# ElesionKyrie/Extreme-Video-Compression-With-Prediction-Using-Pre-trainded-Diffusion-Models-

Hardware: AMD Instinct MI355X
Metric: decoded frames/sec (128x128x30) at q3 (higher is better)
Workload: dtype f32

## Files before the change

### extreme-video-compression-with-prediction-using-pre-trainded-diffusion-models-_amd/build.py

```python
import os
import shutil
import subprocess
import sys
from concurrent.futures import ThreadPoolExecutor

HERE = os.path.dirname(os.path.abspath(__file__))
CSRC = os.path.join(HERE, "csrc")
LIBDIR = os.path.join(HERE, "lib")
OBJDIR = os.path.join(HERE, "build")
INCLUDE = os.path.join(os.path.dirname(HERE), "include")
HIP_SOURCES = ["conv_igemm.hip", "attention.hip", "norm.hip", "fir.hip", "elementwise.hip", "gdn.hip", "stride2.hip", "lpips.hip", "i3d.hip", "frames.hip", "noise.hip", "yuv.hip", "rate.hip", "ssim.hip", "inception.hip", "resample.hip", "tile.hip", "api.hip"]
ARCH = "gfx950"


def _newer(target, deps):
    if not os.path.exists(target):
        return True
    t = os.path.getmtime(target)
    return any(os.path.getmtime(d) > t for d in deps)


def _run(cmd):
    r = subprocess.run(cmd, capture_output=True, text=True)
    if r.returncode != 0:
        raise RuntimeError("build failed: %s\n%s\n%s" % (" ".join(cmd), r.stdout, r.stderr))


def hipcc_path():
    for c in (os.environ.get("HIPCC"), shutil.which("hipcc"), "/opt/rocm/bin/hipcc"):
        if c and os.path.exists(c):
            return c
    raise RuntimeError("hipcc not found (ROCm toolchain required to build libevc_hip.so)")


def build(force=False, verbose=False):
    os.makedirs(LIBDIR, exist_ok=True)
    os.makedirs(OBJDIR, exist_ok=True)
    headers = [os.path.join(INCLUDE, h) for h in ("evc_hip.h", "evc_rans.h")]
    hipcc = hipcc_path()
    flags = ["--offload-arch=" + ARCH, "-O3", "-std=c++17", "-fPIC", "-I", INCLUDE]
    flags += os.environ.get("EVC_HIPCC_FLAGS", "").split()

    def compile_one(src):
        s = os.path.join(CSRC, src)
        o = os.path.join(OBJDIR, src.replace(".hip", ".o"))
        if force or _newer(o, [s] + headers):
            if verbose:
                print("hipcc", src, flush=True)
            _run([hipcc] + flags + ["-c", s, "-o", o])
        return o

    with ThreadPoolExecutor(max_workers=min(6, len(HIP_SOURCES))) as ex:
        objs = list(ex.map(compile_one, HIP_SOURCES))
    hip_so = os.path.join(LIBDIR, "libevc_hip.so")
    if force or _newer(hip_so, objs):
        _run([hipcc, "--offload-arch=" + ARCH, "-shared", "-fPIC", "-o", hip_so] + objs)
    rans_src = os.path.join(CSRC, "rans.cpp")
    rans_so = os.path.join(LIBDIR, "libevc_rans.so")
    if force or _newer(rans_so, [rans_src] + headers):
        _run([shutil.which("g++") or "g++", "-O2", "-std=c++17", "-fPIC", "-shared", "-Wall", "-I", INCLUDE,
              rans_src, "-o", rans_so])
    return hip_so, rans_so


if __name__ == "__main__":
    print(build(force="--force" in sys.argv, verbose=True))
```

### extreme-video-compression-with-prediction-using-pre-trainded-diffusion-models-_amd/csrc/conv_igemm.hip

```cpp
#include <hip/hip_runtime.h>
#include <stdint.h>
#include <stdio.h>
#include "../../include/evc_hip.h"

typedef float f32x16 __attribute__((ext_vector_type(16)));
typedef __attribute__((address_space(3))) void lds_void;
typedef const __attribute__((address_space(1))) void glb_void;

#ifndef EVC_CONV_TAIL
#define EVC_CONV_TAIL 1
#endif
#ifndef EVC_CONV_TM1
#define EVC_CONV_TM1 1
#endif
#ifndef EVC_SPLIT_WIDE_TILES
#define EVC_SPLIT_WIDE_TILES 1
#endif

#ifndef EVC_SPLIT_INTERLEAVE
#define EVC_SPLIT_INTERLEAVE 5
#endif

namespace {

constexpr int BM_MAX = 128;
constexpr int KC = 16;

constexpr int MODE_PLAIN = 0, MODE_AFFINE = 1, MODE_AFFINE_SILU = 2, MODE_SILU = 3, MODE_RELU = 4;

struct ConvK {
    const float* src0; const float* src1; int C0; int C1; int ld0; int ld1;
    const float* coef_a; const float* coef_s;
    const float* w; const float* bias; const float* res; int ld_res;
    float out_scale; int act_out;
    float* out; int ld_out;
    int B, H, W, Co, CoPad, KH, KW;
    int M, HW, nchunk, nsteps, steps_per_split, splits;
    float* ws;
    float* stats;
    const float* w_hdr;
    const unsigned* in_bound;
    int tail_first, tail_splits, tail_sps, tail_rows;
    int cut_chunk;
    const float* x2_src0; const float* x2_src1; int x2_C0, x2_C1, x2_ld0, x2_ld1;
    const char* x2_w;
    const float* x2_hdr;
    const unsigned* x2_bound;
    int bound_stride, generic_epi;
};

__device__ __forceinline__ float bound_scale(unsigned bits) {
    const float b = sqrtf(__uint_as_float(bits));
    if (!(b < 3.0e38f)) return __builtin_nanf("");
    return b > 0.f ? ldexpf(1.0f, 6 - ilogbf(b)) : 1.0f;
}
__device__ __forceinline__ int bound_index(const ConvK& p, int m) { return p.bound_stride ? min(m, p.M - 1) / p.HW : 0; }
__device__ __forceinline__ float in_scale(const ConvK& p, int m) {
    if (!p.in_bound) return 1.0f;
    return bound_scale(p.in_bound[bound_index(p, m)]);
}

__device__ __forceinline__ float silu_f(float v) { return v * __builtin_amdgcn_rcpf(1.0f + __expf(-v)); }

__device__ __forceinline__ float act_fn(float v, int act) {
    if (act == EVC_ACT_SILU) return silu_f(v);
    if (act == EVC_ACT_RELU) return v < 0.f ? 0.f : v;
    return v;
}

template <int MODE>
__device__ __forceinline__ float4 transform(float4 v, const float4& a, const float4& s, bool ok) {
    if (MODE == MODE_AFFINE || MODE == MODE_AFFINE_SILU) {
        v.x = v.x * a.x + s.x; v.y = v.y * a.y + s.y; v.z = v.z * a.z + s.z; v.w = v.w * a.w + s.w;
    }
    if (MODE == MODE_AFFINE_SILU || MODE == MODE_SILU) {
        v.x = silu_f(v.x); v.y = silu_f(v.y); v.z = silu_f(v.z); v.w = silu_f(v.w);
    }
    if (MODE == MODE_RELU) {
        v.x = v.x < 0.f ? 0.f : v.x; v.y = v.y < 0.f ? 0.f : v.y; v.z = v.z < 0.f ? 0.f : v.z; v.w = v.w < 0.f ? 0.f : v.w;
    }
    v.x = ok ? v.x : 0.f; v.y = ok ? v.y : 0.f; v.z = ok ? v.z : 0.f; v.w = ok ? v.w : 0.f;
    return v;
}

template <int TM, int TN>
__device__ __forceinline__ void mfma_group(f32x16 (&acc)[TM][TN], const float4 (&a)[TM], const float4 (&b)[TN]) {
#define EVC_MFMA_E(e)                                                                                   \
    _Pragma("unroll") for (int i = 0; i < TM; ++i) _Pragma("unroll") for (int j = 0; j < TN; ++j)      \
        acc[i][j] = __builtin_amdgcn_mfma_f32_32x32x2f32(a[i].e, b[j].e, acc[i][j], 0, 0, 0);
    EVC_MFMA_E(x) EVC_MFMA_E(y) EVC_MFMA_E(z) EVC_MFMA_E(w)
#undef EVC_MFMA_E
}

template <int TM, int TN, int WM, bool PARTIAL, bool RES, bool STATS, bool ACT>
__device__ __forceinline__ void conv_epilogue_full(const ConvK& p, f32x16 (&acc)[TM][TN], int m0, int n0, int split,
                                                   int wm, int wn, int l31, int half, bool tail) {
    constexpr int BM = 32 * TM * WM;
    const int ws_m0 = tail ? p.tail_first * BM : 0;
    const size_t ws_M = tail ? (size_t)p.tail_rows : (size_t)p.M;
    const float ascale = p.w_hdr ? p.w_hdr[0] / in_scale(p, m0) : 1.0f;
    const float oscale = p.out_scale;
    const int mw = m0 + wm * 32 * TM + 4 * half;
    const int cw = n0 + wn * 32 * TN + l31;
    const bool has_res = RES && (!ACT || p.res != nullptr), has_stats = STATS && (!ACT || p.stats != nullptr);
#pragma unroll
    for (int j = 0; j < TN; ++j) {
        const int co = cw + j * 32;
        const float bias = (!PARTIAL && p.bias) ? p.bias[co] : 0.f;
        float st_sum = 0.f, st_sq = 0.f;
#pragma unroll
        for (int i = 0; i < TM; ++i) {
            const int mb = mw + i * 32;
            if (PARTIAL) {
                float* o = p.ws + ((size_t)split * ws_M + (mb - ws_m0)) * p.Co + co;
#pragma unroll
                for (int r = 0; r < 16; ++r) o[(size_t)((r & 3) + 8 * (r >> 2)) * p.Co] = acc[i][j][r] * ascale;
            } else {
                float rv[16];
#pragma unroll
                for (int r = 0; r < 16; ++r) rv[r] = 0.f;
                if (has_res) {
                    const float* rp = p.res + (size_t)mb * p.ld_res + co;
#pragma unroll
                    for (int r = 0; r < 16; ++r) rv[r] = rp[(size_t)((r & 3) + 8 * (r >> 2)) * p.ld_res];
                }
                float* o = p.out + (size_t)mb * p.ld_out + co;
#pragma unroll
                for (int r = 0; r < 16; ++r) {
                    float v = (acc[i][j][r] * ascale + bias + rv[r]) * oscale;
                    if (ACT) v = act_fn(v, p.act_out);
                    o[(size_t)((r & 3) + 8 * (r >> 2)) * p.ld_out] = v;
                    if (STATS) { st_sum += v; st_sq += v * v; }
                }
            }
        }
        if (has_stats) {
            st_sum += __shfl_xor(st_sum, 32);
            st_sq += __shfl_xor(st_sq, 32);
            if (half == 0) {
                float* sp = p.stats + ((size_t)(m0 / (32 * TM) + wm) * p.Co + co) * 2;
                sp[0] = st_sum; sp[1] = st_sq;
            }
        }
    }
}

template <int TM, int TN, int WM = 2>
__device__ __forceinline__ void conv_epilogue(const ConvK& p, f32x16 (&acc)[TM][TN], int m0, int n0, int split,
                                              int wm, int wn, int l31, int half, bool tail = false) {
    constexpr int BM = 32 * TM * WM;
    constexpr int BN = 64 * TN;
    const bool partial = p.splits > 1 || tail;
    if (!p.generic_epi && m0 + BM <= p.M && n0 + BN <= p.Co) {
#define EVC_EPI(PA, RE, ST, AC) conv_epilogue_full<TM, TN, WM, PA, RE, ST, AC>(p, acc, m0, n0, split, wm, wn, l31, half, tail)
        if (partial) EVC_EPI(true, false, false, false);
        else if (p.act_out != EVC_ACT_NONE) EVC_EPI(false, true, true, true);
        else if (p.res && p.stats) EVC_EPI(false, true, true, false);
        else if (p.stats) EVC_EPI(false, false, true, false);
        else if (p.res) EVC_EPI(false, true, false, false);
        else EVC_EPI(false, false, false, false);
#undef EVC_EPI
        return;
    }
    const int ws_m0 = tail ? p.tail_first * BM : 0;
    const size_t ws_M = tail ? (size_t)p.tail_rows : (size_t)p.M;
    const float ascale = p.w_hdr ? p.w_hdr[0] / in_scale(p, m0) : 1.0f;
    const bool per_row = p.bound_stride && p.in_bound;
    const int mw = m0 + wm * 32 * TM + 4 * half;
    const int cw = n0 + wn * 32 * TN + l31;
    {
#pragma unroll
        for (int j = 0; j < TN; ++j) {
            const int co = cw + j * 32;
            if (co >= p.Co) continue;
            const float bias = (!partial && p.bias) ? p.bias[co] : 0.f;
#pragma unroll
            for (int i = 0; i < TM; ++i) {
#pragma unroll
                for (int r = 0; r < 16; ++r) {
                    const int m = mw + i * 32 + (r & 3) + 8 * (r >> 2);
                    if (m >= p.M) continue;
                    float v = acc[i][j][r] * (per_row ? p.w_hdr[0] / in_scale(p, m) : ascale);
                    if (partial) {
                        p.ws[((size_t)split * ws_M + (m - ws_m0)) * p.Co + co] = v;
                    } else {
                        v += bias;
                        if (p.res) v += p.res[(size_t)m * p.ld_res + co];
                        v *= p.out_scale;
                        p.out[(size_t)m * p.ld_out + co] = act_fn(v, p.act_out);
                    }
                }
            }
        }
    }
}

template <int TM, int TN, int MODE>
__global__ __launch_bounds__(256, 2) void conv_igemm_kernel(ConvK p) {
    constexpr int BM = 64 * TM;
    constexpr int BN = 64 * TN;
    constexpr bool HAS_COEF = MODE == MODE_AFFINE || MODE == MODE_AFFINE_SILU;
    extern __shared__ __attribute__((aligned(16))) float smem[];
    float* const As = smem;
    float* const Ws = smem + 2 * BM * KC;

    const int tid = threadIdx.x;
    const int lane = tid & 63;
    const int wave = tid >> 6;
    const int wm = wave >> 1, wn = wave & 1;
    const int l31 = lane & 31, half = lane >> 5;

    const int m0 = blockIdx.x * BM;
    const int n0 = blockIdx.y * BN;
    const int split = blockIdx.z;
    const int s_begin = split * p.steps_per_split;
    const int s_end = min(p.nsteps, s_begin + p.steps_per_split);

    const int k4 = tid & 3;
    const int padH = p.KH >> 1, padW = p.KW >> 1;
    const int Ct = p.C0 + p.C1;
    unsigned off0[TM], off1[TM], okmask[TM];
    int rb[TM], a_lds[TM];
#pragma unroll
    for (int i = 0; i < TM; ++i) {
        const int row = (tid >> 2) + 64 * i;
        const int m = m0 + row;
        const bool valid = m < p.M;
        const int mm = valid ? m : 0;
        const int b = mm / p.HW;
        const int rem = mm - b * p.HW;
        const int y = rem / p.W;
        const int x = rem - y * p.W;
        rb[i] = b;
        off0[i] = ((unsigned)mm * (unsigned)p.ld0 + 4u * k4) * 4u;
        off1[i] = ((unsigned)mm * (unsigned)p.ld1 + 4u * k4) * 4u;
        unsigned mask = 0;
        for (int ty = 0; ty < p.KH; ++ty)
            for (int tx = 0; tx < p.KW; ++tx) {
                const int yy = y + ty - padH, xx = x + tx - padW;
                const bool ok = valid && yy >= 0 && yy < p.H && xx >= 0 && xx < p.W;
                mask |= (ok ? 1u : 0u) << (ty * p.KW + tx);
            }
        okmask[i] = mask;
        a_lds[i] = row * KC + 4 * (k4 ^ ((row >> 2) & 3));
    }

    const int fsw = (l31 >> 2) & 3;
    const int rd0 = 4 * ((0 + half) ^ fsw), rd1 = 4 * ((2 + half) ^ fsw);
    const int a_rd = (wm * 32 * TM + l31) * KC, w_rd = (wn * 32 * TN + l31) * KC;

    int c_chunk, c_ty, c_tx;
    {
        const int taps = p.KH * p.KW;
        c_chunk = s_begin / taps;
        const int tap = s_begin - c_chunk * taps;
        c_ty = tap / p.KW;
        c_tx = tap - c_ty * p.KW;
    }
    float4 areg[TM], ca[TM], cs[TM];
    bool aok[TM];

    auto load_coefs = [&]() {
        if (HAS_COEF) {
#pragma unroll
            for (int i = 0; i < TM; ++i) {
                const size_t co = (size_t)rb[i] * Ct + c_chunk * KC + 4 * k4;
                ca[i] = *reinterpret_cast<const float4*>(p.coef_a + co);
                cs[i] = *reinterpret_cast<const float4*>(p.coef_s + co);
            }
        }
    };
    auto issue_loads = [&](int buf) {
        const int c = c_chunk * KC;
        const bool first = c < p.C0;
        const char* src = reinterpret_cast<const char*>(first ? p.src0 : p.src1);
        const int ld = first ? p.ld0 : p.ld1;
        const int tap = c_ty * p.KW + c_tx;
        const int delta = (((c_ty - padH) * p.W + (c_tx - padW)) * ld + (first ? c : c - p.C0)) * 4;
        const unsigned safe = (unsigned)((first ? c : c - p.C0) + 4 * k4) * 4u;
#pragma unroll
        for (int i = 0; i < TM; ++i) {
            aok[i] = (okmask[i] >> tap) & 1u;
            const unsigned o = aok[i] ? (first ? off0[i] : off1[i]) + (unsigned)delta : safe;
            areg[i] = *reinterpret_cast<const float4*>(src + o);
        }
        const float* wt = p.w + ((size_t)(tap * p.nchunk + c_chunk) * p.CoPad + n0) * KC;
        float* wl = Ws + buf * BN * KC;
#pragma unroll
        for (int j = 0; j < TN; ++j)
            __builtin_amdgcn_global_load_lds((glb_void*)(wt + (size_t)(tid + 256 * j) * 4),
                                             (lds_void*)(wl + (wave * 16 + 64 * j) * KC), 16, 0, 0);
    };
    auto advance = [&]() {
        ++c_tx;
        if (c_tx == p.KW) { c_tx = 0; ++c_ty; }
        if (c_ty == p.KH) { c_ty = 0; ++c_chunk; }
    };
    auto store_a = [&](int buf) {
        float* A = As + buf * BM * KC;
#pragma unroll
        for (int i = 0; i < TM; ++i)
            *reinterpret_cast<float4*>(A + a_lds[i]) = transform<MODE>(areg[i], ca[i], cs[i], aok[i]);
    };

    f32x16 acc[TM][TN];
#pragma unroll
    for (int i = 0; i < TM; ++i)
#pragma unroll
        for (int j = 0; j < TN; ++j)
#pragma unroll
            for (int r = 0; r < 16; ++r) acc[i][j][r] = 0.f;

    if (s_begin < s_end) {
        load_coefs();
        issue_loads(0);
        store_a(0);
    }
    __syncthreads();

    for (int s = s_begin; s < s_end; ++s) {
        const int buf = (s - s_begin) & 1;
        if (s + 1 < s_end) {
            const int prev_chunk = c_chunk;
            advance();
            if (HAS_COEF && c_chunk != prev_chunk) load_coefs();
        }
        issue_loads(buf ^ 1);

        const float* Ab = As + buf * BM * KC + a_rd;
        const float* Wb = Ws + buf * BN * KC + w_rd;
        float4 a0[TM], b0[TN], a1[TM], b1[TN];
#pragma unroll
        for (int i = 0; i < TM; ++i) a0[i] = *reinterpret_cast<const float4*>(Ab + i * 32 * KC + rd0);
#pragma unroll
        for (int j = 0; j < TN; ++j) b0[j] = *reinterpret_cast<const float4*>(Wb + j * 32 * KC + rd0);
#pragma unroll
        for (int i = 0; i < TM; ++i) a1[i] = *reinterpret_cast<const float4*>(Ab + i * 32 * KC + rd1);
#pragma unroll
        for (int j = 0; j < TN; ++j) b1[j] = *reinterpret_cast<const float4*>(Wb + j * 32 * KC + rd1);
        mfma_group<TM, TN>(acc, a0, b0);
        __builtin_amdgcn_sched_barrier(0);
        store_a(buf ^ 1);
        mfma_group<TM, TN>(acc, a1, b1);
        __syncthreads();
    }

    conv_epilogue<TM, TN>(p, acc, m0, n0, split, wm, wn, l31, half);
}

typedef __bf16 bf16x8 __attribute__((ext_vector_type(8)));
typedef _Float16 f16x8 __attribute__((ext_vector_type(8)));

__device__ __forceinline__ void split3_bf16(const float4& v0, const float4& v1, bf16x8& p1, bf16x8& p2, bf16x8& p3) {
    const float x[8] = {v0.x, v0.y, v0.z, v0.w, v1.x, v1.y, v1.z, v1.w};
#pragma unroll
    for (int j = 0; j < 8; ++j) {
        const __bf16 a = (__bf16)x[j];
        const float r = x[j] - (float)a;
        const __bf16 b = (__bf16)r;
        p1[j] = a; p2[j] = b; p3[j] = (__bf16)(r - (float)b);
    }
}

constexpr float F16_ACT_SCALE = 8.0f;

__device__ __forceinline__ void split2_f16(const float4& v0, const float4& v1, float xscale, f16x8& p1, f16x8& p2) {
    const float x[8] = {v0.x, v0.y, v0.z, v0.w, v1.x, v1.y, v1.z, v1.w};
#pragma unroll
    for (int j = 0; j < 8; ++j) {
        const float v = x[j] * xscale;
        const _Float16 a = (_Float16)v;
        p1[j] = a; p2[j] = (_Float16)(v - (float)a);
    }
}

template <int NP> struct Split;
template <> struct Split<3> {
    typedef bf16x8 vec;
    static constexpr int NTERM = 6;
    static __device__ __forceinline__ constexpr int qa(int t) { return t == 0 ? 2 : (t == 1 || t == 3) ? 1 : 0; }
    static __device__ __forceinline__ constexpr int qb(int t) { return t == 2 ? 2 : (t == 1 || t == 4) ? 1 : 0; }
    static __device__ __forceinline__ f32x16 mfma(const vec& a, const vec& b, const f32x16& c) {
        return __builtin_amdgcn_mfma_f32_32x32x16_bf16(a, b, c, 0, 0, 0);
    }
    static __device__ __forceinline__ void split(const float4& v0, const float4& v1, float, vec (&pl)[3]) {
        split3_bf16(v0, v1, pl[0], pl[1], pl[2]);
    }
};
template <> struct Split<2> {
    typedef f16x8 vec;
    static constexpr int NTERM = 3;
    static __device__ __forceinline__ constexpr int qa(int t) { return t == 0 ? 1 : 0; }
    static __device__ __forceinline__ constexpr int qb(int t) { return t == 1 ? 1 : 0; }
    static __device__ __forceinline__ f32x16 mfma(const vec& a, const vec& b, const f32x16& c) {
        return __builtin_amdgcn_mfma_f32_32x32x16_f16(a, b, c, 0, 0, 0);
    }
    static __device__ __forceinline__ void split(const float4& v0, const float4& v1, float xscale, vec (&pl)[2]) {
        split2_f16(v0, v1, xscale, pl[0], pl[1]);
    }
};

template <int NP, int TM, int TN, int MODE>
__global__ __launch_bounds__(256, 2) void conv_splitn_kernel(ConvK p) {
    typedef Split<NP> SP;
    typedef typename SP::vec vec;
    constexpr int BM = 64 * TM;
    constexpr int BN = 64 * TN;
    constexpr int RB = 32;
    constexpr int NPIECE = NP * 2 * TN;
    constexpr int NWD = (NPIECE + 3) / 4;
    constexpr bool HAS_COEF = MODE == MODE_AFFINE || MODE == MODE_AFFINE_SILU;
    extern __shared__ __attribute__((aligned(16))) char smem_b[];
    char* const As = smem_b;
    char* const Ws = smem_b + 2 * NP * BM * RB;

    const int tid = threadIdx.x;
    const int lane = tid & 63;
    const int wave = __builtin_amdgcn_readfirstlane(tid >> 6);
    const int wm = wave >> 1, wn = wave & 1;
    const int l31 = lane & 31, half = lane >> 5;

    const int m0 = blockIdx.x * BM;
    const int n0 = blockIdx.y * BN;
    const int split = blockIdx.z;
    const int s_begin = split * p.steps_per_split;
    const int s_end = min(p.nsteps, s_begin + p.steps_per_split);

    const int row = tid >> 1, kh = tid & 1;
    const bool a_active = TM == 2 || wave < 2;
    const int padH = p.KH >> 1, padW = p.KW >> 1;
    const int Ct = p.C0 + p.C1;
    unsigned off0, off1, okmask = 0;
    int rb;
    {
        const int m = m0 + row;
        const bool valid = a_active && m < p.M;
        const int mm = valid ? m : 0;
        const int b = mm / p.HW;
        const int rem = mm - b * p.HW;
        const int y = rem / p.W;
        const int x = rem - y * p.W;
        rb = b;
        off0 = ((unsigned)mm * (unsigned)p.ld0 + 8u * kh) * 4u;
        off1 = ((unsigned)mm * (unsigned)p.ld1 + 8u * kh) * 4u;
        for (int ty = 0; ty < p.KH; ++ty)
            for (int tx = 0; tx < p.KW; ++tx) {
                const int yy = y + ty - padH, xx = x + tx - padW;
                const bool ok = valid && yy >= 0 && yy < p.H && xx >= 0 && xx < p.W;
                okmask |= (ok ? 1u : 0u) << (ty * p.KW + tx);
            }
    }
    const int a_lds = row * RB + 16 * (kh ^ ((row >> 3) & 1));
    const int fr = l31 * RB + 16 * (half ^ ((l31 >> 3) & 1));
    const int a_rd = wm * 32 * TM * RB + fr, w_rd = wn * 32 * TN * RB + fr;

    unsigned wsrc[NWD];
    int wdst[NWD];
#pragma unroll
    for (int j = 0; j < NWD; ++j) {
        const int idx = min(wave + 4 * j, NPIECE - 1);
        const int part = idx / (2 * TN), seg = idx - part * (2 * TN);
        wsrc[j] = (unsigned)((part * p.CoPad + n0 + seg * 32) * RB + lane * 16);
        wdst[j] = (part * BN + seg * 32) * RB;
    }
    const unsigned slab = (unsigned)NP * (unsigned)p.CoPad * RB;
    const unsigned w_tap = (unsigned)p.nchunk * slab;
    const unsigned w_wrap = slab - (unsigned)(p.KH * p.KW) * w_tap;

    int c_chunk, c_ty, c_tx;
    {
        const int taps = p.KH * p.KW;
        c_chunk = s_begin / taps;
        const int tap = s_begin - c_chunk * taps;
        c_ty = tap / p.KW;
        c_tx = tap - c_ty * p.KW;
    }
    unsigned w_off = (unsigned)((c_ty * p.KW + c_tx) * p.nchunk + c_chunk) * slab;
    const char* a_src; int a_px, a_delta; unsigned a_safe; bool a_first;
    auto chunk_setup = [&]() {
        const int c = c_chunk * KC;
        a_first = c < p.C0;
        a_src = reinterpret_cast<const char*>(a_first ? p.src0 : p.src1);
        a_px = (a_first ? p.ld0 : p.ld1) * 4;
        const int cc = a_first ? c : c - p.C0;
        a_delta = ((c_ty - padH) * p.W + (c_tx - padW)) * a_px + cc * 4;
        a_safe = (unsigned)(cc + 8 * kh) * 4u;
    };
    float4 areg[2] = {}, ca[2], cs[2];
    bool aok = false;
    const float xscale = F16_ACT_SCALE * in_scale(p, m0 + row);
    auto load_coefs = [&]() {
        if (HAS_COEF) {
            const size_t co = (size_t)rb * Ct + c_chunk * KC + 8 * kh;
            ca[0] = *reinterpret_cast<const float4*>(p.coef_a + co);
            ca[1] = *reinterpret_cast<const float4*>(p.coef_a + co + 4);
            cs[0] = *reinterpret_cast<const float4*>(p.coef_s + co);
            cs[1] = *reinterpret_cast<const float4*>(p.coef_s + co + 4);
        }
    };
    auto issue_loads = [&](int buf) {
        if (a_active) {
            aok = (okmask >> (c_ty * p.KW + c_tx)) & 1u;
            const unsigned o = aok ? (a_first ? off0 : off1) + (unsigned)a_delta : a_safe;
            areg[0] = *reinterpret_cast<const float4*>(a_src + o);
            areg[1] = *reinterpret_cast<const float4*>(a_src + o + 16);
        }
        const char* wt = reinterpret_cast<const char*>(p.w) + w_off;
        char* wl = Ws + buf * NP * BN * RB;
#pragma unroll
        for (int j = 0; j < NWD; ++j)
            __builtin_amdgcn_global_load_lds((glb_void*)(wt + wsrc[j]), (lds_void*)(wl + wdst[j]), 16, 0, 0);
    };
    auto advance = [&]() -> bool {
        ++c_tx; a_delta += a_px; w_off += w_tap;
        if (c_tx == p.KW) { c_tx = 0; ++c_ty; a_delta += (p.W - p.KW) * a_px; }
        if (c_ty == p.KH) { c_ty = 0; ++c_chunk; w_off += w_wrap; chunk_setup(); return true; }
        return false;
    };
    auto store_a = [&](int buf) {
        if (!a_active) return;
        vec pl[NP];
        SP::split(transform<MODE>(areg[0], ca[0], cs[0], aok), transform<MODE>(areg[1], ca[1], cs[1], aok), xscale, pl);
        char* A = As + buf * NP * BM * RB + a_lds;
#pragma unroll
        for (int q = 0; q < NP; ++q) *reinterpret_cast<vec*>(A + q * BM * RB) = pl[q];
    };

    f32x16 acc[TM][TN];
#pragma unroll
    for (int i = 0; i < TM; ++i)
#pragma unroll
        for (int j = 0; j < TN; ++j)
#pragma unroll
            for (int r = 0; r < 16; ++r) acc[i][j][r] = 0.f;

    chunk_setup();
    if (s_begin < s_end) {
        load_coefs();
        issue_loads(0);
        store_a(0);
    }
    __syncthreads();

    for (int s = s_begin; s < s_end; ++s) {
        const int buf = (s - s_begin) & 1;
        if (s + 1 < s_end) {
            if (advance() && HAS_COEF) load_coefs();
        }
        issue_loads(buf ^ 1);

        const char* Ab = As + buf * NP * BM * RB + a_rd;
        const char* Wb = Ws + buf * NP * BN * RB + w_rd;
        vec a[TM][NP], b[TN][NP];
// ... 76 lines not shown
    int wdst[NWD];
#pragma unroll
    for (int j = 0; j < NWD; ++j) {
        const int idx = min(wave + 4 * j, 6 * TN - 1);
        const int part = idx / (2 * TN), seg = idx - part * (2 * TN);
        wsrc[j] = (unsigned)((part * p.CoPad + n0 + seg * 32) * RB + lane * 16);
        wdst[j] = (part * BN + seg * 32) * RB;
    }
    const unsigned slab = 3u * (unsigned)p.CoPad * RB;
    const unsigned w_tap = (unsigned)p.nchunk * slab;
    const unsigned w_wrap = slab - (unsigned)(p.KH * p.KW) * w_tap;

    int w_ty, w_tx, l_chunk, l_ty, l_tx;
    {
        const int taps = p.KH * p.KW;
        l_chunk = s_begin / taps;
        const int tap = s_begin - l_chunk * taps;
        l_ty = w_ty = tap / p.KW;
        l_tx = w_tx = tap - l_ty * p.KW;
    }
    unsigned w_off = (unsigned)((w_ty * p.KW + w_tx) * p.nchunk + l_chunk) * slab;
    const char* a_src; int a_px, a_delta; unsigned a_safe; bool a_first;
    auto chunk_setup = [&]() {
        const int c = l_chunk * KC;
        a_first = c < p.C0;
        a_src = reinterpret_cast<const char*>(a_first ? p.src0 : p.src1);
        a_px = (a_first ? p.ld0 : p.ld1) * 4;
        const int cc = a_first ? c : c - p.C0;
        a_delta = ((l_ty - padH) * p.W + (l_tx - padW)) * a_px + cc * 4;
        a_safe = (unsigned)(cc + 8 * kh) * 4u;
    };
    float4 areg[2] = {}, ca[2], cs[2];
    bool aok = false;
    auto load_coefs = [&]() {
        if (HAS_COEF) {
            const size_t co = (size_t)rb * Ct + l_chunk * KC + 8 * kh;
            ca[0] = *reinterpret_cast<const float4*>(p.coef_a + co);
            ca[1] = *reinterpret_cast<const float4*>(p.coef_a + co + 4);
            cs[0] = *reinterpret_cast<const float4*>(p.coef_s + co);
            cs[1] = *reinterpret_cast<const float4*>(p.coef_s + co + 4);
        }
    };
    auto load_a = [&]() {
        if (a_active) {
            aok = (okmask >> (l_ty * p.KW + l_tx)) & 1u;
            const unsigned o = aok ? (a_first ? off0 : off1) + (unsigned)a_delta : a_safe;
            areg[0] = *reinterpret_cast<const float4*>(a_src + o);
            areg[1] = *reinterpret_cast<const float4*>(a_src + o + 16);
        }
    };
    auto dma_w = [&](int buf) {
        const char* wt = reinterpret_cast<const char*>(p.w) + w_off;
        char* wl = Ws + buf * 3 * BN * RB;
#pragma unroll
        for (int j = 0; j < NWD; ++j)
            __builtin_amdgcn_global_load_lds((glb_void*)(wt + wsrc[j]), (lds_void*)(wl + wdst[j]), 16, 0, 0);
    };
    auto advance_w = [&]() {
        ++w_tx; w_off += w_tap;
        if (w_tx == p.KW) { w_tx = 0; ++w_ty; }
        if (w_ty == p.KH) { w_ty = 0; w_off += w_wrap; }
    };
    auto advance_l = [&]() {
        ++l_tx; a_delta += a_px;
        if (l_tx == p.KW) { l_tx = 0; ++l_ty; a_delta += (p.W - p.KW) * a_px; }
        if (l_ty == p.KH) { l_ty = 0; ++l_chunk; chunk_setup(); load_coefs(); }
    };
    auto store_a = [&](int buf) {
        if (!a_active) return;
        bf16x8 p1, p2, p3;
        split3_bf16(transform<MODE>(areg[0], ca[0], cs[0], aok), transform<MODE>(areg[1], ca[1], cs[1], aok), p1, p2, p3);
        char* A = As + buf * 3 * BM * RB + a_lds;
        *reinterpret_cast<bf16x8*>(A) = p1;
        *reinterpret_cast<bf16x8*>(A + BM * RB) = p2;
        *reinterpret_cast<bf16x8*>(A + 2 * BM * RB) = p3;
    };

    f32x16 acc[TM][TN];
#pragma unroll
    for (int i = 0; i < TM; ++i)
#pragma unroll
        for (int j = 0; j < TN; ++j)
#pragma unroll
            for (int r = 0; r < 16; ++r) acc[i][j][r] = 0.f;

    bf16x8 a[TM][3], b[TN][3], bp[TN];
    if (nst > 0) {
        chunk_setup();
        load_coefs();
        load_a();
        dma_w(0);
        store_a(0);
        if (1 < nst) { advance_l(); advance_w(); }
        load_a();
        dma_w(1);
        store_a(1);
        if (2 < nst) { advance_l(); advance_w(); }
        load_a();
        __syncthreads();
#pragma unroll
        for (int i = 0; i < TM; ++i) a[i][2] = *reinterpret_cast<const bf16x8*>(As + a_rd + (2 * BM + i * 32) * RB);
#pragma unroll
        for (int j = 0; j < TN; ++j) bp[j] = *reinterpret_cast<const bf16x8*>(Ws + w_rd + (0 * BN + j * 32) * RB);
    }

#define EVC_SPLIT_TERM(qa, qb)                                                                          \
    _Pragma("unroll") for (int i = 0; i < TM; ++i) _Pragma("unroll") for (int j = 0; j < TN; ++j)      \
        acc[i][j] = __builtin_amdgcn_mfma_f32_32x32x16_bf16(a[i][qa], b[j][qb], acc[i][j], 0, 0, 0);
    for (int t = 0; t < nst; ++t) {
        const int cur = t & 1;
        const char* Ab = As + cur * 3 * BM * RB + a_rd;
        const char* Wb = Ws + cur * 3 * BN * RB + w_rd;
#pragma unroll
        for (int j = 0; j < TN; ++j) b[j][0] = bp[j];
#pragma unroll
        for (int i = 0; i < TM; ++i) a[i][1] = *reinterpret_cast<const bf16x8*>(Ab + (1 * BM + i * 32) * RB);
#pragma unroll
        for (int j = 0; j < TN; ++j) b[j][1] = *reinterpret_cast<const bf16x8*>(Wb + (1 * BN + j * 32) * RB);
#pragma unroll
        for (int i = 0; i < TM; ++i) a[i][0] = *reinterpret_cast<const bf16x8*>(Ab + (0 * BM + i * 32) * RB);
#pragma unroll
        for (int j = 0; j < TN; ++j) b[j][2] = *reinterpret_cast<const bf16x8*>(Wb + (2 * BN + j * 32) * RB);
        EVC_SPLIT_TERM(2, 0) EVC_SPLIT_TERM(1, 1) EVC_SPLIT_TERM(0, 2)
        __builtin_amdgcn_sched_barrier(0);
        if (a_active) asm volatile("s_waitcnt vmcnt(2) lgkmcnt(0)\n\ts_barrier" ::: "memory");
        else asm volatile("s_waitcnt vmcnt(0) lgkmcnt(0)\n\ts_barrier" ::: "memory");
        __builtin_amdgcn_sched_barrier(0);
        dma_w(cur);
        const char* An = As + (cur ^ 1) * 3 * BM * RB + a_rd;
        const char* Wn = Ws + (cur ^ 1) * 3 * BN * RB + w_rd;
#pragma unroll
        for (int i = 0; i < TM; ++i) a[i][2] = *reinterpret_cast<const bf16x8*>(An + (2 * BM + i * 32) * RB);
#pragma unroll
        for (int j = 0; j < TN; ++j) bp[j] = *reinterpret_cast<const bf16x8*>(Wn + (0 * BN + j * 32) * RB);
        store_a(cur);
        EVC_SPLIT_TERM(1, 0) EVC_SPLIT_TERM(0, 1) EVC_SPLIT_TERM(0, 0)
#if EVC_SPLIT_INTERLEAVE
        __builtin_amdgcn_sched_group_barrier(0x010, NWD, 0);
        __builtin_amdgcn_sched_group_barrier(0x100, TM + TN, 0);
#pragma unroll
        for (int g = 0; g < 6 * TM * TN / 2; ++g) {
            __builtin_amdgcn_sched_group_barrier(0x008, 1, 0);
            __builtin_amdgcn_sched_group_barrier(0x002, EVC_SPLIT_INTERLEAVE, 0);
        }
#endif
        __builtin_amdgcn_sched_barrier(0);
        if (t + 3 < nst) { advance_w(); advance_l(); }
        load_a();
    }
#undef EVC_SPLIT_TERM

    conv_epilogue<TM, TN>(p, acc, m0, n0, split, wm, wn, l31, half);
}


template <int NP, int WM, int TN, int MODE>
__global__ __launch_bounds__(128 * WM, WM == 2 ? 2 : 1) void conv_split_rr_kernel(ConvK p) {
    typedef Split<NP> SP;
    typedef typename SP::vec vec;
    constexpr int TM = 2;
    constexpr int BM = 64 * WM;
    constexpr int NT = 128 * WM;
    constexpr int BN = 64 * TN;
    constexpr int RB = 32;
    constexpr int NPIECE = NP * 2 * TN;
    constexpr int NWD = WM == 2 ? (NPIECE + 3) / 4 : TN;
    constexpr bool HAS_COEF = MODE == MODE_AFFINE || MODE == MODE_AFFINE_SILU;
    extern __shared__ __attribute__((aligned(16))) char smem_b[];
    const int SR = (BM / p.W) * (p.W + 2);
    const int APL = SR * RB;
    char* const As = smem_b;
    char* const Ws = smem_b + 2 * NP * APL;

    const int tid = threadIdx.x;
    const int lane = tid & 63;
    const int wave = __builtin_amdgcn_readfirstlane(tid >> 6);
    const int wm = wave >> 1, wn = wave & 1;
    const int l31 = lane & 31, half = lane >> 5;

    const bool tail = WM == 2 && (int)blockIdx.x >= p.tail_first;
    const int tq = tail ? ((int)blockIdx.x - p.tail_first) / p.tail_splits : 0;
    const int m0 = (tail ? p.tail_first + tq : (int)blockIdx.x) * BM;
    const int n0 = blockIdx.y * BN;
    const int split = tail ? (int)blockIdx.x - p.tail_first - tq * p.tail_splits : (int)blockIdx.z;
    const int sps = tail ? p.tail_sps : p.steps_per_split;
    const int s_begin = split * sps;
    const int nst = min(p.nsteps, s_begin + sps) - s_begin;
    const int nmac = nst / 3;

    const int row = tid >> 1, kh = tid & 1;
    const int Ct = p.C0 + p.C1;
    unsigned off0, off1, okrow = 0;
    int rb;
    {
        const int m = m0 + row;
        const bool valid = m < p.M;
        const int mm = valid ? m : 0;
        const int b = mm / p.HW;
        const int rem = mm - b * p.HW;
        const int y = rem / p.W;
        rb = b;
        off0 = ((unsigned)mm * (unsigned)p.ld0 + 8u * kh) * 4u;
        off1 = ((unsigned)mm * (unsigned)p.ld1 + 8u * kh) * 4u;
#pragma unroll
        for (int ty = 0; ty < 3; ++ty) {
            const int yy = y + ty - 1;
            okrow |= ((valid && yy >= 0 && yy < p.H) ? 1u : 0u) << ty;
        }
    }
    const int srow_p = row + 2 * (row / p.W) + 1;
    const int a_lds = srow_p * RB + 16 * (kh ^ ((srow_p >> 3) & 1));
    int ard[TM][3];
#pragma unroll
    for (int i = 0; i < TM; ++i) {
        const int ml = wm * 32 * TM + i * 32 + l31;
        const int base = ml + 2 * (ml / p.W);
#pragma unroll
        for (int tx = 0; tx < 3; ++tx) {
            const int sr = base + tx;
            ard[i][tx] = sr * RB + 16 * (half ^ ((sr >> 3) & 1));
        }
    }
    const int w_rd = wn * 32 * TN * RB + l31 * RB + 16 * (half ^ ((l31 >> 3) & 1));

    unsigned wsrc[NWD];
    int wdst[NWD];
    const bool w_active = WM == 2 || wave < 2 * NP;
#pragma unroll
    for (int j = 0; j < NWD; ++j) {
        const int idx = WM == 2 ? min(wave + 4 * j, NPIECE - 1) : min(wave * TN + j, NPIECE - 1);
        const int part = idx / (2 * TN), seg = idx - part * (2 * TN);
        wsrc[j] = (unsigned)((part * p.CoPad + n0 + seg * 32) * RB + lane * 16);
        wdst[j] = (part * BN + seg * 32) * RB;
    }
    const unsigned slab = (unsigned)NP * (unsigned)p.CoPad * RB;
    const unsigned w_tap = (unsigned)p.nchunk * slab;
    const unsigned w_wrap = slab - 9u * w_tap;

    int l_chunk = s_begin / 9;
    int l_ty = (s_begin - l_chunk * 9) / 3;
    int w_ty = l_ty, w_tx = 0;
    unsigned w_off = (unsigned)((w_ty * 3) * p.nchunk + l_chunk) * slab;
    const char* a_src; int a_rowb, a_delta; bool a_first;
    unsigned a_safe;
    auto chunk_setup = [&]() {
        const int c = l_chunk * KC;
        a_first = c < p.C0;
        a_src = reinterpret_cast<const char*>(a_first ? p.src0 : p.src1);
        a_rowb = (a_first ? p.ld0 : p.ld1) * 4 * p.W;
        const int cc = a_first ? c : c - p.C0;
        a_delta = (l_ty - 1) * a_rowb + cc * 4;
        a_safe = (unsigned)(cc + 8 * kh) * 4u;
    };
    float4 areg[2], ca[2], cs[2];
    bool aok = false;
    auto load_coefs = [&]() {
        if (HAS_COEF) {
            const size_t co = (size_t)rb * Ct + l_chunk * KC + 8 * kh;
            ca[0] = *reinterpret_cast<const float4*>(p.coef_a + co);
            ca[1] = *reinterpret_cast<const float4*>(p.coef_a + co + 4);
            cs[0] = *reinterpret_cast<const float4*>(p.coef_s + co);
            cs[1] = *reinterpret_cast<const float4*>(p.coef_s + co + 4);
        }
    };
    auto load_a = [&]() {
        aok = (okrow >> l_ty) & 1u;
        const unsigned o = aok ? (a_first ? off0 : off1) + (unsigned)a_delta : a_safe;
        areg[0] = *reinterpret_cast<const float4*>(a_src + o);
        areg[1] = *reinterpret_cast<const float4*>(a_src + o + 16);
    };
    auto advance_l = [&]() {
        ++l_ty; a_delta += a_rowb;
        if (l_ty == 3) { l_ty = 0; ++l_chunk; chunk_setup(); load_coefs(); }
    };
    auto dma_w = [&](int wb) {
        const char* wt = reinterpret_cast<const char*>(p.w) + w_off;
        char* wl = Ws + wb * NP * BN * RB;
        if (w_active) {
#pragma unroll
            for (int j = 0; j < NWD; ++j)
                __builtin_amdgcn_global_load_lds((glb_void*)(wt + wsrc[j]), (lds_void*)(wl + wdst[j]), 16, 0, 0);
        }
    };
    auto advance_w = [&]() {
        ++w_tx; w_off += w_tap;
        if (w_tx == 3) { w_tx = 0; ++w_ty; }
        if (w_ty == 3) { w_ty = 0; w_off += w_wrap; }
    };
    const float xscale = F16_ACT_SCALE * in_scale(p, m0);
    auto store_a = [&](int ab) {
        vec pl[NP];
        SP::split(transform<MODE>(areg[0], ca[0], cs[0], aok), transform<MODE>(areg[1], ca[1], cs[1], aok), xscale, pl);
        char* A = As + ab * NP * APL + a_lds;
#pragma unroll
        for (int q = 0; q < NP; ++q) *reinterpret_cast<vec*>(A + q * APL) = pl[q];
    };

    f32x16 acc[TM][TN];
#pragma unroll
    for (int i = 0; i < TM; ++i)
#pragma unroll
        for (int j = 0; j < TN; ++j)
#pragma unroll
            for (int r = 0; r < 16; ++r) acc[i][j][r] = 0.f;

    for (int o = tid * 16; o < 2 * NP * APL; o += NT * 16) *reinterpret_cast<float4*>(As + o) = make_float4(0.f, 0.f, 0.f, 0.f);
    __syncthreads();
// ... 553 lines not shown
            else if (!(EVC_WIDE_ABL & 2)) load_b(b[(T + EVC_WIDE_BDIST) % 3], (T + EVC_WIDE_BDIST < 9) ? c : cn, (T + EVC_WIDE_BDIST) % 9); \
            if (T == 0 && !(EVC_WIDE_ABL & 8)) coef_load(cn);                                           \
            if constexpr (LOADK >= 0 && LOADK < NU && !(EVC_WIDE_ABL & 8)) stage_load(LOADK < 0 ? 0 : LOADK, cn); \
            const char* An = (T == 8) ? Anxt : Acur;                    \
            const int toff = tap_off((T + 1) % 9);                                                      \
            _Pragma("unroll") for (int i = 0; i < TM; ++i) {                                            \
                EVC_PIN(a[i][0]); EVC_PIN(a[i][1]);                                                     \
                EVC_WIDE_MFMA_I(i, b[T % 3])                                                            \
                if (!(EVC_WIDE_ABL & 4)) read_a(i, An, toff);                                           \
            }                                                                                           \
            if constexpr (STOREK >= 0 && STOREK < NU && !(EVC_WIDE_ABL & 1)) stage_store(STOREK < 0 ? 0 : STOREK, ab ^ 1); \
             \
             \
            _Pragma("unroll") for (int m = 0; m < 36; ++m) {                                            \
                if (m % EVC_WIDE_VMEM_EVERY == 0) __builtin_amdgcn_sched_group_barrier(0x020, 1, 0);    \
                __builtin_amdgcn_sched_group_barrier(0x008, 1, 0);                                      \
                __builtin_amdgcn_sched_group_barrier(0x402, 4, 0);                                      \
                if (m % 9 == 8) __builtin_amdgcn_sched_group_barrier(0x100, 2, 0);                      \
            }                                                                                           \
            __builtin_amdgcn_sched_group_barrier(0x200, 2, 0);                                          \
            __builtin_amdgcn_sched_barrier(0);                                                          \
            TAIL_CODE                                                                                   \
            __builtin_amdgcn_sched_barrier(0);                                                          \
        }
        EVC_WIDE_STEP(0, 0, -1, )
        EVC_WIDE_STEP(1, 1, -1, )
        EVC_WIDE_STEP(2, 2, 0, )
        EVC_WIDE_STEP(3, 3, 1, )
        EVC_WIDE_STEP(4, -1, 2, )
        EVC_WIDE_STEP(5, -1, 3, )
        EVC_WIDE_STEP(6, -1, -1, )
        EVC_WIDE_STEP(7, -1, -1, asm volatile("s_waitcnt lgkmcnt(0)\n\ts_barrier" ::: "memory");)
        EVC_WIDE_STEP(8, -1, -1, )
#undef EVC_WIDE_STEP
    }
#undef EVC_WIDE_MFMA_I
#undef EVC_PIN
#undef EVC_PIN4

    if (EVC_WIDE_ABL & 16) {
        float sacc = 0.f;
#pragma unroll
        for (int i = 0; i < TM; ++i)
#pragma unroll
            for (int j = 0; j < TN; ++j)
#pragma unroll
                for (int e = 0; e < 16; ++e) sacc += acc[i][j][e];
        p.out[(size_t)m0 * p.ld_out + tid] = sacc;
        return;
    }
    EVC_STAMP(2)
    __syncthreads();
    wide_epilogue(p, acc, As, (EVC_WIDE_ABL & 128) ? 0 : m0, n0, split, wave, lane, tail);
#ifdef EVC_WIDE_STAMPS
    asm volatile("s_waitcnt vmcnt(0)" ::: "memory");
    EVC_STAMP(3)
    if (threadIdx.x == 0) g_wide_stamps[(blockIdx.x & 8191) * 8 + 4] = __builtin_amdgcn_s_getreg(6 | (8 << 6) | (3 << 11)) ;
#endif
}

__global__ __launch_bounds__(1024) void conv_splitk_reduce_kernel(const float* __restrict__ ws, int splits, int M,
                                                                  int Co, const float* __restrict__ bias,
                                                                  const float* __restrict__ res, int ld_res,
                                                                  float scale, int act, float* __restrict__ out,
                                                                  int ld_out, float* __restrict__ stats) {
    __shared__ float red[2][16][64];
    const int l = threadIdx.x & 63;
    const int c = blockIdx.y * 64 + l;
    const int rg = threadIdx.x >> 6;
    const int m_base = blockIdx.x * 64;
    const size_t total = (size_t)M * Co;
    float s_sum = 0.f, s_sq = 0.f;
    if (c < Co) {
        const float b = bias ? bias[c] : 0.f;
        float v[4];
        size_t idx[4];
        bool ok[4];
#pragma unroll
        for (int k = 0; k < 4; ++k) {
            const int m = m_base + rg + 16 * k;
            ok[k] = m < M;
            idx[k] = (size_t)(ok[k] ? m : 0) * Co + c;
            v[k] = 0.f;
        }
        for (int z = 0; z < splits; ++z) {
            const float* w = ws + (size_t)z * total;
#pragma unroll
            for (int k = 0; k < 4; ++k) v[k] += w[idx[k]];
        }
#pragma unroll
        for (int k = 0; k < 4; ++k) {
            if (!ok[k]) continue;
            const int m = m_base + rg + 16 * k;
            float o = v[k] + b;
            if (res) o += res[(size_t)m * ld_res + c];
            o = act_fn(o * scale, act);
            out[(size_t)m * ld_out + c] = o;
            s_sum += o; s_sq += o * o;
        }
    }
    if (stats) {
        red[0][rg][l] = s_sum;
        red[1][rg][l] = s_sq;
        __syncthreads();
        if (rg == 0 && c < Co) {
            float a = 0.f, q = 0.f;
#pragma unroll
            for (int k = 0; k < 16; ++k) { a += red[0][k][l]; q += red[1][k][l]; }
            float* sp = stats + ((size_t)blockIdx.x * Co + c) * 2;
            sp[0] = a; sp[1] = q;
        }
    }
}

__global__ void conv_pack_weights_kernel(const float* w, float* packed, int Co, int CoPad, int Ci, int KH, int KW) {
    const int taps = KH * KW, nchunk = Ci / KC;
    const size_t total = (size_t)taps * nchunk * CoPad * KC;
    for (size_t i = (size_t)blockIdx.x * blockDim.x + threadIdx.x; i < total; i += (size_t)gridDim.x * blockDim.x) {
        const int k = (int)(i % KC);
        size_t t = i / KC;
        const int co = (int)(t % CoPad); t /= CoPad;
        const int chunk = (int)(t % nchunk);
        const int tap = (int)(t / nchunk);
        const int kl = (((k >> 2) ^ ((co >> 2) & 3)) << 2) | (k & 3);
        float v = 0.f;
        if (co < Co) v = w[((size_t)co * Ci + chunk * KC + kl) * taps + tap];
        packed[i] = v;
    }
}

__global__ void conv_pack_split_kernel(const float* w, __bf16* packed, int Co, int CoPad, int Ci, int KH, int KW) {
    const int taps = KH * KW, nchunk = Ci / KC;
    const size_t total = (size_t)taps * nchunk * CoPad * KC;
    for (size_t i = (size_t)blockIdx.x * blockDim.x + threadIdx.x; i < total; i += (size_t)gridDim.x * blockDim.x) {
        const int k = (int)(i % KC);
        size_t t = i / KC;
        const int co = (int)(t % CoPad); t /= CoPad;
        const int chunk = (int)(t % nchunk);
        const int tap = (int)(t / nchunk);
        float v = 0.f;
        if (co < Co) v = w[((size_t)co * Ci + chunk * KC + k) * taps + tap];
        const __bf16 a = (__bf16)v;
        const float r = v - (float)a;
        const __bf16 b = (__bf16)r;
        const __bf16 c = (__bf16)(r - (float)b);
        const int pos = (((k >> 3) ^ ((co >> 3) & 1)) << 3) | (k & 7);
        const size_t base = (size_t)(tap * nchunk + chunk) * 3 * CoPad * KC;
        packed[base + ((size_t)0 * CoPad + co) * KC + pos] = a;
        packed[base + ((size_t)1 * CoPad + co) * KC + pos] = b;
        packed[base + ((size_t)2 * CoPad + co) * KC + pos] = c;
    }
}

constexpr int F16_HDR_BYTES = 256;

__global__ void conv_absmax_kernel(const float* w, size_t n, unsigned* out_bits) {
    float m = 0.f;
    for (size_t i = (size_t)blockIdx.x * blockDim.x + threadIdx.x; i < n; i += (size_t)gridDim.x * blockDim.x)
        m = fmaxf(m, fabsf(w[i]));
    for (int o = 32; o > 0; o >>= 1) m = fmaxf(m, __shfl_xor(m, o));
    if ((threadIdx.x & 63) == 0 && m > 0.f) atomicMax(out_bits, __float_as_uint(m));
}

__device__ __forceinline__ float f16_weight_scale(unsigned max_bits) {
    const float mx = __uint_as_float(max_bits);
    if (!(mx > 0.f) || !isfinite(mx)) return 1.0f;
    return ldexpf(1.0f, 14 - ilogbf(mx));
}

__global__ void conv_pack_f16_kernel(const float* w, char* packed, int Co, int CoPad, int Ci, int KH, int KW) {
    const int taps = KH * KW, nchunk = Ci / KC;
    const size_t total = (size_t)taps * nchunk * CoPad * KC;
    float* hdr = reinterpret_cast<float*>(packed);
    const float sw = f16_weight_scale(reinterpret_cast<const unsigned*>(packed)[2]);
    _Float16* body = reinterpret_cast<_Float16*>(packed + F16_HDR_BYTES);
    if (blockIdx.x == 0 && threadIdx.x == 0) { hdr[0] = 1.0f / (F16_ACT_SCALE * sw); hdr[1] = sw; }
    for (size_t i = (size_t)blockIdx.x * blockDim.x + threadIdx.x; i < total; i += (size_t)gridDim.x * blockDim.x) {
        const int k = (int)(i % KC);
        size_t t = i / KC;
        const int co = (int)(t % CoPad); t /= CoPad;
        const int chunk = (int)(t % nchunk);
        const int tap = (int)(t / nchunk);
        float v = 0.f;
        if (co < Co) v = w[((size_t)co * Ci + chunk * KC + k) * taps + tap] * sw;
        const _Float16 a = (_Float16)v;
        const _Float16 b = (_Float16)(v - (float)a);
        const int pos = (((k >> 3) ^ ((co >> 3) & 1)) << 3) | (k & 7);
        const size_t base = (size_t)(tap * nchunk + chunk) * 2 * CoPad * KC;
        body[base + ((size_t)0 * CoPad + co) * KC + pos] = a;
        body[base + ((size_t)1 * CoPad + co) * KC + pos] = b;
    }
}

int pick_tn(int CoPad) {
    if (CoPad % 192 == 0) return 3;
    if (CoPad % 128 == 0) return 2;
    return 1;
}

}

extern "C" int evc_conv_co_pad(int Co) { return (Co + 63) / 64 * 64; }

extern "C" long long evc_conv_packed_floats(int Co, int Ci, int KH, int KW) {
    return (long long)KH * KW * (Ci / KC) * evc_conv_co_pad(Co) * KC;
}

extern "C" int evc_conv_pack_weights_f32(const float* w, float* packed, int Co, int Ci, int KH, int KW, void* stream) {
    if (!w || !packed || Co <= 0 || Ci <= 0 || Ci % KC != 0 || KH <= 0 || KW <= 0) return EVC_EINVAL;
    const long long total = evc_conv_packed_floats(Co, Ci, KH, KW);
    int grid = (int)((total + 255) / 256 > 4096 ? 4096 : (total + 255) / 256);
    hipLaunchKernelGGL(conv_pack_weights_kernel, dim3(grid), dim3(256), 0, (hipStream_t)stream, w, packed, Co,
                       evc_conv_co_pad(Co), Ci, KH, KW);
    return hipGetLastError() == hipSuccess ? EVC_OK : EVC_ELAUNCH;
}

extern "C" long long evc_conv_packed_bytes(int Co, int Ci, int KH, int KW, int arith) {
    const long long elems = evc_conv_packed_floats(Co, Ci, KH, KW);
    switch (arith) {
        case EVC_ARITH_F32: return elems * 4;
        case EVC_ARITH_BF16X6: return elems * 6;
        case EVC_ARITH_F16X3: return F16_HDR_BYTES + elems * 4;
        default: return EVC_EINVAL;
    }
}

extern "C" int evc_conv_pack_weights(const float* w, void* packed, int Co, int Ci, int KH, int KW, int arith,
                                     void* stream) {
    if (arith == EVC_ARITH_F32) return evc_conv_pack_weights_f32(w, (float*)packed, Co, Ci, KH, KW, stream);
    if (arith != EVC_ARITH_BF16X6 && arith != EVC_ARITH_F16X3) return EVC_EINVAL;
    if (!w || !packed || Co <= 0 || Ci <= 0 || Ci % KC != 0 || KH <= 0 || KW <= 0) return EVC_EINVAL;
    const long long total = evc_conv_packed_floats(Co, Ci, KH, KW);
    int grid = (int)((total + 255) / 256 > 4096 ? 4096 : (total + 255) / 256);
    hipStream_t st = (hipStream_t)stream;
    if (arith == EVC_ARITH_BF16X6) {
        hipLaunchKernelGGL(conv_pack_split_kernel, dim3(grid), dim3(256), 0, st, w, (__bf16*)packed, Co,
                           evc_conv_co_pad(Co), Ci, KH, KW);
    } else {
        if (hipMemsetAsync(packed, 0, F16_HDR_BYTES, st) != hipSuccess) return EVC_ELAUNCH;
        const size_t n = (size_t)Co * Ci * KH * KW;
        hipLaunchKernelGGL(conv_absmax_kernel, dim3(grid), dim3(256), 0, st, w, n, reinterpret_cast<unsigned*>(packed) + 2);
        hipLaunchKernelGGL(conv_pack_f16_kernel, dim3(grid), dim3(256), 0, st, w, (char*)packed, Co,
                           evc_conv_co_pad(Co), Ci, KH, KW);
    }
    return hipGetLastError() == hipSuccess ? EVC_OK : EVC_ELAUNCH;
}

static int conv_validate(const evc_conv_args* a) {
    if (!a || !a->src0 || !a->w_packed || !a->out) return EVC_EINVAL;
    if (a->C0 <= 0 || a->C0 % KC != 0 || a->C1 < 0 || a->C1 % KC != 0) return EVC_EINVAL;
    if (a->C1 > 0 && !a->src1) return EVC_EINVAL;
    if ((a->ld0 != 0 && (a->ld0 < a->C0 || (a->ld0 & 3))) || (a->ld1 != 0 && (a->ld1 < a->C1 || (a->ld1 & 3))))
        return EVC_EINVAL;
    if ((a->coef_a == nullptr) != (a->coef_s == nullptr)) return EVC_EINVAL;
    if (a->B <= 0 || a->H <= 0 || a->W <= 0 || a->Co <= 0) return EVC_EINVAL;
    if (a->KH <= 0 || a->KW <= 0 || !(a->KH & 1) || !(a->KW & 1)) return EVC_EINVAL;
    if (a->ld_out < a->Co || (a->res && a->ld_res < a->Co)) return EVC_EINVAL;
    if ((long long)a->B * a->H * a->W > 0x7fffffffLL) return EVC_EINVAL;
    if (a->arith != EVC_ARITH_F32 && a->arith != EVC_ARITH_BF16X6 && a->arith != EVC_ARITH_F16X3) return EVC_EINVAL;
    if (a->x2_w_packed) {
        if (!a->x2_src0 || !a->x2_bound || a->x2_C0 <= 0 || a->x2_C0 % KC != 0 || a->x2_C1 < 0 || a->x2_C1 % KC != 0) return EVC_EINVAL;
        if (a->x2_C1 > 0 && !a->x2_src1) return EVC_EINVAL;
        if ((a->x2_ld0 != 0 && (a->x2_ld0 < a->x2_C0 || (a->x2_ld0 & 3))) || (a->x2_ld1 != 0 && (a->x2_ld1 < a->x2_C1 || (a->x2_ld1 & 3))))
            return EVC_EINVAL;
    }
    return EVC_OK;
}

struct TileCfg { int tm, tn, bm, bn; long long tiles; int splits = 1; int reuse = 0; int wide = 0; int steps_per_split;
                 int tail_first = 0, tail_tiles = 0, tail_splits = 1, tail_sps = 0;
                 int cut_chunk = 0;
                 void set_wide(long long wgs) { *this = TileCfg(); wide = 1; tm = 4; tn = 3; bm = 256; bn = 192; tiles = wgs; } };
static int g_wide_cut = 1;
static int g_tail_split = EVC_CONV_TAIL;
static int g_wide_tiles = EVC_SPLIT_WIDE_TILES;
static int g_no_reuse = 0;
static int g_wide_mid = 1;
static int g_wide256 = 1;
static int g_force_tm = 0;

static void split_tile_cfg(const evc_conv_args* a, long long M, long long ntile, int nsteps, TileCfg& c, bool rr_ok, bool inv) {
    const double K = (double)a->KH * a->KW * (a->C0 + a->C1);
    const bool f16 = a->arith == EVC_ARITH_F16X3 && rr_ok;
    const double E = f16 ? 20.0 : 6.0, F2 = f16 ? 1.5 : 1.0;
    const auto grid_time = [&](long long n, double sps) {
        const long long R = n / 512, rem = n - R * 512;
        return (sps + E) * ((double)R * F2 + (rem == 0 ? 0.0 : (rem <= 256 && f16 ? 1.0 : F2)));
    };
    double best = 1e300;
    int best_tm = 2, best_s = 1;
    for (int tm = 2; tm >= 1; --tm) {
        if (!inv && g_force_tm && tm != g_force_tm) continue;
        const long long tiles = ((M + 64 * tm - 1) / (64 * tm)) * ntile;
        const int smax = a->splits > 0 ? a->splits : (nsteps / 4 < 1 ? 1 : (nsteps / 4 > 32 ? 32 : nsteps / 4));
        for (int s = a->splits > 0 ? a->splits : 1; s <= smax; ++s) {
            const double sps = (double)((nsteps + s - 1) / s);
            const double slab_mb = (double)s * (double)M * a->Co * 4.0 / 1e6;
            const double pen = s > 1 ? 1.0 + (slab_mb > 192.0 ? 300.0 : 40.0) * s / K : 1.0;
            const double tmf = tm == 1 ? (a->KH * a->KW > 1 ? 0.5 / (rr_ok ? 0.55 : 0.75) : 0.5) : 1.0;
            const double t = grid_time(tiles * s, sps) * pen * tmf;
            if (t < best * 0.9999) { best = t; best_tm = tm; best_s = s; }
        }
    }
    c.tm = best_tm;
    c.bm = 64 * c.tm;
    c.tiles = ((M + c.bm - 1) / c.bm) * ntile;
    c.splits = best_s;
    if (!inv && rr_ok && g_tail_split && a->splits <= 0 && !g_force_tm && M % 128 == 0) {
// ... 454 lines not shown
```

### extreme-video-compression-with-prediction-using-pre-trainded-diffusion-models-_amd/lib.py

```python
import ctypes
import math
import os
from ctypes import POINTER, c_char_p, c_double, c_float, c_int, c_int32, c_longlong, c_uint, c_uint8, c_ulonglong, c_void_p

import numpy as np
import torch

HERE = os.path.dirname(os.path.abspath(__file__))
HIP_SO = os.path.join(HERE, "lib", "libevc_hip.so")
if os.environ.get("EVC_HIP_SO"):
    HIP_SO = os.path.abspath(os.environ["EVC_HIP_SO"])
RANS_SO = os.path.join(HERE, "lib", "libevc_rans.so")

ACT_NONE, ACT_SILU, ACT_RELU = 0, 1, 2
ARITH_F32, ARITH_BF16X6, ARITH_F16X3 = 0, 1, 2
_ARITH_NAMES = {"f32": ARITH_F32, "bf16x6": ARITH_BF16X6, "f16x3": ARITH_F16X3}
_ARITH_DTYPES = {ARITH_F32: torch.float32, ARITH_BF16X6: torch.bfloat16, ARITH_F16X3: torch.float16}


def _arith_policy():
    name = os.environ.get("EVC_CONV_ARITH", "f16x3").lower()
    if name not in _ARITH_NAMES:
        raise ValueError(f"EVC_CONV_ARITH must be one of {sorted(_ARITH_NAMES)}, got {name!r}")
    return _ARITH_NAMES[name]


def default_arith():
    a = _arith_policy()
    return ARITH_BF16X6 if a == ARITH_F16X3 else a


def bounded_arith():
    return _arith_policy()


class EvcLibraryError(RuntimeError):
    pass


class EvcKernelError(RuntimeError):
    pass


class ConvArgs(ctypes.Structure):
    _fields_ = [("src0", c_void_p), ("src1", c_void_p), ("C0", c_int), ("C1", c_int),
                ("ld0", c_int), ("ld1", c_int),
                ("coef_a", c_void_p), ("coef_s", c_void_p), ("act_in", c_int),
                ("w_packed", c_void_p), ("bias", c_void_p), ("res", c_void_p), ("ld_res", c_int),
                ("out_scale", c_float), ("act_out", c_int),
                ("out", c_void_p), ("ld_out", c_int),
                ("B", c_int), ("H", c_int), ("W", c_int), ("Co", c_int), ("KH", c_int), ("KW", c_int),
                ("splits", c_int), ("stats_out", c_void_p), ("arith", c_int), ("in_bound", c_void_p),
                ("x2_src0", c_void_p), ("x2_src1", c_void_p), ("x2_C0", c_int), ("x2_C1", c_int), ("x2_ld0", c_int),
                ("x2_ld1", c_int), ("x2_w_packed", c_void_p), ("x2_bound", c_void_p), ("invariant", c_int)]


class ConvPlan(ctypes.Structure):
    _fields_ = [("kernel", ctypes.c_char * 96), ("tile_m", c_int), ("tile_n", c_int), ("splits", c_int),
                ("steps_per_split", c_int), ("cut_chunk", c_int), ("tail_tiles", c_int), ("tail_splits", c_int),
                ("stats_runs", c_int), ("fused_1x1", c_int)]


class AttentionPlan(ctypes.Structure):
    _fields_ = [("kernel", ctypes.c_char * 64), ("waves", c_int), ("kparts", c_int), ("tiles_per_part", c_int),
                ("kv_planes", c_int), ("merge", c_int), ("short_seq", c_int),
                ("lds_bytes", c_longlong), ("parts_bytes", c_longlong), ("ws_bytes", c_longlong)]


HIP_SYMBOLS = {
    "evc_version": (c_char_p, []),
    "evc_arch": (c_char_p, []),
    "evc_device_ok": (c_int, []),
    "evc_clock_probe": (c_int, [c_void_p, c_int, c_void_p, c_void_p]),
    "evc_im2col_nchw_f32": (c_int, [c_void_p, c_void_p] + [c_int] * 9 + [c_void_p, c_void_p, c_void_p]),
    "evc_maxpool3s2_nhwc_f32": (c_int, [c_void_p, c_void_p, c_int, c_int, c_int, c_int, c_void_p]),
    "evc_lpips_layer_f32": (c_int, [c_void_p, c_void_p, c_void_p, c_void_p, c_int, c_int, c_int, c_int, c_void_p]),
    "evc_maxpool2d_nhwc_f32": (c_int, [c_void_p, c_void_p] + [c_int] * 7 + [c_void_p]),
    "evc_lpips_map_f32": (c_int, [c_void_p, c_void_p, c_void_p, c_void_p, c_int, c_int, c_int, c_void_p]),
    "evc_lpips_map_mean_f32": (c_int, [c_void_p, c_void_p, c_int, c_int, c_int, c_void_p]),
    "evc_lpips_upsample_add_f32": (c_int, [c_void_p, c_void_p] + [c_int] * 6 + [c_void_p]),
    "evc_i3d_stem_im2col_f32": (c_int, [c_void_p, c_void_p] + [c_int] * 17 + [c_void_p]),
    "evc_maxpool3d_same_nthwc_f32": (c_int, [c_void_p, c_void_p] + [c_int] * 11 + [c_void_p]),
    "evc_i3d_head_f32": (c_int, [c_void_p] * 4 + [c_int] * 6 + [c_void_p]),
    "evc_upfirdn2d_f32": (c_int, [c_void_p, c_void_p, POINTER(c_float)] + [c_int] * 13 + [c_void_p]),
    "evc_upfirdn2d_nhwc_f32": (c_int, [c_void_p, c_void_p, POINTER(c_float)] + [c_int] * 10 +
                               [c_void_p, c_void_p, c_int, c_void_p]),
    "evc_pack_nchw_to_nhwc_f32": (c_int, [c_void_p, c_int, c_void_p, c_int, c_void_p, c_int, c_int, c_int, c_int,
                                          c_void_p]),
    "evc_nhwc_to_nchw_f32": (c_int, [c_void_p, c_int, c_void_p, c_int, c_int, c_int, c_int, c_void_p]),
    "evc_chan_stats_f32": (c_int, [c_void_p, c_void_p, c_int, c_int, c_int, c_int, c_void_p]),
    "evc_gn_coeffs_f32": (c_int, [c_void_p, c_int, c_int, c_void_p, c_int, c_int, c_int, c_int, c_int, c_float,
                                  c_int, c_void_p, c_void_p, c_void_p, c_int, c_void_p, c_void_p, c_void_p,
                                  c_void_p]),
    "evc_gn_coeffs_bound_f32": (c_int, [c_void_p, c_int, c_int, c_void_p, c_int, c_int, c_int, c_int, c_int, c_float,
                                        c_int, c_void_p, c_void_p, c_void_p, c_int, c_void_p, c_void_p, c_void_p,
                                        c_void_p, c_void_p, c_void_p]),
    "evc_moments_bound_f32": (c_int, [c_void_p, c_int, c_int, c_int, c_int, c_int, c_int, c_void_p, c_void_p, c_void_p]),
    "evc_gn_coeffs_site_f32": (c_int, [c_void_p, c_int, c_int, c_void_p, c_int, c_int, c_int, c_int, c_int, c_float,
                                       c_int, c_void_p, c_void_p, c_void_p, c_int, c_void_p, c_void_p, c_void_p,
                                       c_void_p, c_void_p, c_int, c_void_p]),
    "evc_gn_coeffs_bound_site_f32": (c_int, [c_void_p, c_int, c_int, c_void_p, c_int, c_int, c_int, c_int, c_int, c_float,
                                             c_int, c_void_p, c_void_p, c_void_p, c_int, c_void_p, c_void_p, c_void_p,
                                             c_void_p, c_void_p, c_void_p, c_int, c_void_p]),
    "evc_moments_bound_site_f32": (c_int, [c_void_p, c_int, c_int, c_int, c_int, c_int, c_int, c_void_p, c_void_p, c_void_p,
                                           c_int, c_void_p]),
    "evc_invariant_plan_revision": (c_int, []),
    "evc_conv_plan_query": (c_int, [POINTER(ConvArgs), POINTER(ConvPlan)]),
    "evc_gn_coeffs_bound_sample_f32": (c_int, [c_void_p, c_int, c_int, c_void_p, c_int, c_int, c_int, c_int, c_int, c_float,
                                               c_int, c_void_p, c_void_p, c_void_p, c_int, c_void_p, c_void_p, c_void_p,
                                               c_void_p, c_void_p, c_void_p, c_int, c_void_p]),
    "evc_moments_bound_sample_f32": (c_int, [c_void_p, c_int, c_int, c_int, c_int, c_int, c_int, c_void_p, c_void_p, c_void_p,
                                             c_int, c_void_p]),
    "evc_attention_invariant_workspace_bytes": (c_longlong, [c_int, c_int, c_int, c_int]),
    "evc_attention_invariant_f32": (c_int, [c_void_p, c_void_p, c_void_p, c_int, c_void_p, c_int, c_int, c_int, c_int, c_int,
                                            c_float, c_void_p, c_void_p, c_void_p]),
    "evc_attention_f16x3_f32": (c_int, [c_void_p, c_void_p, c_void_p, c_int, c_void_p, c_int, c_int, c_int, c_int, c_int,
                                        c_float, c_void_p, c_void_p, c_void_p]),
    "evc_deconv5x5s2_phase_weights_f32": (c_int, [c_void_p, c_void_p, c_int, c_int, c_int, c_int, c_void_p]),
    "evc_conv5x5s2_phase_weights_f32": (c_int, [c_void_p, c_void_p, c_int, c_int, c_int, c_void_p]),
    "evc_depth_to_space2_f32": (c_int, [c_void_p, c_int, c_int, c_void_p, c_int, c_int, c_int, c_int, c_void_p]),
    "evc_space_to_depth2_f32": (c_int, [c_void_p, c_int, c_int, c_void_p, c_int, c_int, c_int, c_int, c_int, c_void_p]),
    "evc_deconv5x5s2_workspace_bytes": (c_longlong, [c_int, c_int, c_int, c_int]),
    "evc_deconv5x5s2_f32": (c_int, [c_void_p, c_void_p, c_int, c_void_p, c_void_p, c_void_p] + [c_int] * 6 + [c_void_p]),
    "evc_conv5x5s2_workspace_bytes": (c_longlong, [c_int, c_int, c_int, c_int]),
    "evc_conv5x5s2_f32": (c_int, [c_void_p, c_int, c_void_p, c_int, c_void_p, c_void_p, c_void_p] + [c_int] * 6 + [c_void_p]),
    "evc_gdn_workspace_bytes": (c_longlong, [c_int, c_int, c_int, c_int]),
    "evc_gdn_f32": (c_int, [c_void_p, c_void_p, c_int, c_void_p, c_void_p, c_void_p, c_int, c_int, c_int, c_int, c_int,
                            c_int, c_void_p]),
    "evc_affine_act_nhwc_f32": (c_int, [c_void_p, c_void_p, c_void_p, c_void_p, c_int, c_int, c_int, c_int, c_int,
                                        c_int, c_void_p]),
    "evc_conv_co_pad": (c_int, [c_int]),
    "evc_conv_packed_floats": (c_longlong, [c_int, c_int, c_int, c_int]),
    "evc_conv_pack_weights_f32": (c_int, [c_void_p, c_void_p, c_int, c_int, c_int, c_int, c_void_p]),
    "evc_conv_packed_bytes": (c_longlong, [c_int, c_int, c_int, c_int, c_int]),
    "evc_conv_pack_weights": (c_int, [c_void_p, c_void_p, c_int, c_int, c_int, c_int, c_int, c_void_p]),
    "evc_conv_set_option": (c_int, [c_char_p, c_int]),
    "evc_spade_act_nhwc_f32": (c_int, [c_void_p, c_void_p, c_void_p, c_void_p, c_int, c_void_p, c_void_p, c_int, c_void_p,
                                       c_void_p, c_int, c_void_p, c_int, c_int, c_int, c_int, c_int, c_void_p]),
    "evc_conv_choose_splits": (c_int, [POINTER(ConvArgs)]),
    "evc_conv_kernel_name": (c_int, [POINTER(ConvArgs), c_char_p, c_int]),
    "evc_conv_fused_1x1_supported": (c_int, [POINTER(ConvArgs)]),
    "evc_conv_stats_splits": (c_int, [POINTER(ConvArgs)]),
    "evc_conv_workspace_bytes": (c_longlong, [POINTER(ConvArgs)]),
    "evc_conv2d_nhwc_f32": (c_int, [POINTER(ConvArgs), c_void_p, c_void_p]),
    "evc_conv2d_nhwc_profiled_f32": (c_int, [POINTER(ConvArgs), c_void_p, c_void_p, c_void_p, c_void_p]),
    "evc_attention_f32": (c_int, [c_void_p, c_void_p, c_void_p, c_int, c_void_p, c_int, c_int, c_int, c_int, c_int,
                                  c_float, c_void_p]),
    "evc_attention_workspace_bytes": (c_longlong, [c_int, c_int, c_int, c_int]),
    "evc_attention_set_option": (c_int, [c_char_p, c_int]),
    "evc_attention_plan_query": (c_int, [c_int, c_int, c_int, c_int, c_int, c_int, c_int, POINTER(AttentionPlan)]),
    "evc_attention_ws_f32": (c_int, [c_void_p, c_void_p, c_void_p, c_int, c_void_p, c_int, c_int, c_int, c_int, c_int,
                                     c_float, c_void_p, c_void_p]),
    "evc_frame_group_norm_f32": (c_int, [c_void_p] * 4 + [c_int] * 5 + [c_float, c_void_p]),
    "evc_frame_attention_f32": (c_int, [c_void_p, c_int, c_void_p, c_int] + [c_int] * 5 + [c_float, c_void_p]),
    "evc_frame_mix_f32": (c_int, [c_void_p] * 4 + [c_int] * 3 + [c_longlong, c_void_p]),
    "evc_frame_taps_f32": (c_int, [c_void_p, c_void_p] + [c_int] * 4 + [c_void_p]),
    "evc_ddpm_step_f32": (c_int, [c_void_p, c_void_p, c_void_p, c_longlong] + [c_float] * 5 + [c_int, c_void_p]),
    "evc_ddim_step_f32": (c_int, [c_void_p, c_void_p, c_longlong] + [c_float] * 4 + [c_int, c_void_p]),
    "evc_axpy_f32": (c_int, [c_void_p, c_void_p, c_void_p, c_longlong, c_float, c_void_p]),
    "evc_pndm_transfer_f32": (c_int, [c_void_p, c_void_p, c_void_p, c_longlong, c_float, c_float, c_float, c_int,
                                      c_void_p]),
    "evc_lincomb4_f32": (c_int, [c_void_p] * 5 + [c_longlong] + [c_float] * 4 + [c_void_p]),
    "evc_scale_clamp_f32": (c_int, [c_void_p, c_void_p, c_longlong, c_float, c_float, c_int, c_float, c_float,
                                    c_void_p]),
    "evc_gate_residual_f32": (c_int, [c_void_p, c_void_p, c_void_p, c_void_p, c_longlong, c_void_p]),
    "evc_elic_gather_params_f32": (c_int, [c_void_p] + [c_int] * 8 + [c_void_p, c_int, c_void_p, c_void_p,
                                                                       c_void_p]),
    "evc_elic_scatter_symbols_f32": (c_int, [c_void_p, c_void_p, c_void_p] + [c_int] * 7 + [c_void_p]),
    "evc_elic_quantize_f32": (c_int, [c_void_p, c_int, c_int, c_void_p] + [c_int] * 5 + [c_void_p, c_void_p]),
    "evc_elic_rate_pass_f32": (c_int, [c_void_p] + [c_int] * 4 + [c_void_p] + [c_int] * 6 + [c_void_p, c_void_p, c_void_p]),
    "evc_bottleneck_rate_f32": (c_int, [c_void_p] + [c_int] * 5 + [c_void_p] * 5),
    "evc_noise_normal_f32": (c_int, [c_void_p, c_void_p, c_int, c_longlong, c_ulonglong, c_uint, c_int, c_void_p]),
    "evc_yuv420_to_rgb": (c_int, [c_void_p] + [c_longlong] * 6 + [c_int] * 5 + [c_void_p, c_int, c_void_p]),
    "evc_rgb_to_yuv420": (c_int, [c_void_p, c_void_p] + [c_longlong] * 6 + [c_int] * 4 + [c_void_p, c_void_p]),
    "evc_resample_h_u8": (c_int, [c_void_p, c_int, c_int, c_int, c_longlong, c_longlong, c_void_p, c_void_p, c_int, c_int, c_void_p,
                                  c_void_p]),
    "evc_resample_v_u8": (c_int, [c_void_p, c_int, c_int, c_int, c_longlong, c_longlong, c_void_p, c_void_p, c_int, c_int, c_void_p,
                                  c_void_p]),
    "evc_tile_grid_check": (c_int, [c_int] * 6 + [c_void_p, c_void_p, c_int]),
    "evc_tile_gather_u8": (c_int, [c_void_p] + [c_int] * 6 + [c_void_p] * 6),
    "evc_tile_blend_f32": (c_int, [c_void_p] + [c_int] * 6 + [c_void_p] * 6),
    "evc_ssim_workspace_bytes": (c_longlong, [c_int, c_int, c_int]),
    "evc_ssim_planes_f32": (c_int, [c_void_p, c_void_p, c_int, c_int, c_int, c_void_p, c_double, c_double, c_void_p, c_void_p,
                                    c_void_p]),
    "evc_inception_stem_im2col_f32": (c_int, [c_void_p, c_void_p] + [c_int] * 7 + [c_void_p]),
    "evc_im2col_nhwc_f32": (c_int, [c_void_p, c_void_p] + [c_int] * 11 + [c_void_p]),
    "evc_pool3x3s1p1_nhwc_f32": (c_int, [c_void_p, c_void_p] + [c_int] * 5 + [c_void_p]),
    "evc_spatial_mean_nhwc_f32": (c_int, [c_void_p, c_void_p] + [c_int] * 3 + [c_void_p]),
    "evc_knn_radius_f32": (c_int, [c_void_p, c_void_p] + [c_int] * 3 + [c_void_p]),
    "evc_manifold_hits_f32": (c_int, [c_void_p] * 4 + [c_int] * 3 + [c_void_p]),
}

RANS_SYMBOLS = {
    "evc_rans_version": (c_char_p, []),
    "evc_rans_max_encoded_bytes": (c_longlong, [c_longlong]),
    "evc_rans_encode_with_indexes": (c_longlong, [POINTER(c_int32), POINTER(c_int32), c_longlong, POINTER(c_int32),
                                                  c_int, POINTER(c_int32), POINTER(c_int32), c_int,
                                                  POINTER(c_uint8), c_longlong]),
    "evc_rans_decode_with_indexes": (c_int, [POINTER(c_uint8), c_longlong, POINTER(c_int32), c_longlong,
                                             POINTER(c_int32), c_int, POINTER(c_int32), POINTER(c_int32), c_int,
                                             POINTER(c_int32)]),
    "evc_pmf_to_quantized_cdf": (c_int, [POINTER(c_float), c_int, c_int, POINTER(c_int32)]),
}

_hip = None
_rans = None


def _load(path, symbols, what):
    if not os.path.exists(path):
        raise EvcLibraryError(f"{what} not built: {path} is missing. Run `python -c \"import __graft_entry__ as g; "
                              f"g.build()\"` (needs hipcc / g++). There is no fallback path.")
    lib = ctypes.CDLL(path)
    for name, (res, args) in symbols.items():
        try:
            fn = getattr(lib, name)
        except AttributeError as e:
            raise EvcLibraryError(f"{path} does not export {name}") from e
        fn.restype = res
        fn.argtypes = args
    return lib


def hip_lib(require_device=True):
    global _hip
    if _hip is None:
        _hip = _load(HIP_SO, HIP_SYMBOLS, "libevc_hip.so")
        for item in filter(None, os.environ.get("EVC_CONV_OPTIONS", "").split(",")):
            name, _, value = item.partition("=")
            if _hip.evc_conv_set_option(name.strip().encode(), int(value or 1)) != 0:
                raise ValueError(f"EVC_CONV_OPTIONS: unknown convolution option {name!r}")
    if require_device:
        if not torch.cuda.is_available():
            raise EvcLibraryError("no HIP device visible: the evc_amd compute path is gfx950-only (no CPU fallback)")
        if not getattr(hip_lib, "_checked", False):
            if _hip.evc_device_ok() != 1:
                raise EvcLibraryError("current HIP device is not gfx950 (MI355X); libevc_hip.so has no code for it")
            hip_lib._checked = True
    return _hip


def rans_lib():
    global _rans
    if _rans is None:
        _rans = _load(RANS_SO, RANS_SYMBOLS, "libevc_rans.so")
    return _rans


def _check(rc, name):
    if rc != 0:
        raise EvcKernelError(f"{name} failed with code {rc} "
                             "(-1 invalid argument, -2 unsupported, -3 launch failure)")


def stream_ptr():
    return c_void_p(torch.cuda.current_stream().cuda_stream)


def ptr(t):
    if t is None:
        return None
    assert t.is_cuda and t.is_contiguous(), "device-contiguous tensor required"
    return c_void_p(t.data_ptr())


def fptr(t, dtype=torch.float32):
    assert t is None or t.dtype == dtype, (t.dtype, dtype)
    return ptr(t)



def upfirdn2d_nchw(x, kernel, up=1, down=1, pad=(0, 0)):
    L = hip_lib()
    assert x.dim() == 4 and x.dtype == torch.float32
    x = x.contiguous()
    n, c, h, w = x.shape
    k = np.ascontiguousarray(np.asarray(kernel.detach().cpu() if torch.is_tensor(kernel) else kernel,
                                        dtype=np.float32))
    kh, kw = k.shape
    oh = (h * up + pad[0] + pad[1] - kh) // down + 1
    ow = (w * up + pad[0] + pad[1] - kw) // down + 1
    out = torch.empty((n, c, oh, ow), device=x.device, dtype=torch.float32)
    _check(L.evc_upfirdn2d_f32(fptr(x), fptr(out), k.ctypes.data_as(POINTER(c_float)), n * c, h, w, kh, kw, up, up,
                               down, down, pad[0], pad[1], pad[0], pad[1], stream_ptr()), "evc_upfirdn2d_f32")
    return out


def upfirdn2d_nhwc(x, kernel, up, down, pad, coef=None, act=ACT_NONE, out=None):
    L = hip_lib()
    B, H, W, C = x.shape
    k = np.ascontiguousarray(np.asarray(kernel, dtype=np.float32))
    kh, kw = k.shape
    oh = (H * up + pad[0] + pad[1] - kh) // down + 1
    ow = (W * up + pad[0] + pad[1] - kw) // down + 1
    if out is None:
        out = torch.empty((B, oh, ow, C), device=x.device, dtype=torch.float32)
    ca, cs = coef if coef is not None else (None, None)
    _check(L.evc_upfirdn2d_nhwc_f32(fptr(x), fptr(out), k.ctypes.data_as(POINTER(c_float)), B, H, W, C, kh, kw, up,
# ... 397 lines not shown
    if nbytes < 0:
        raise EvcKernelError(f"evc_conv_packed_bytes rejected the arguments ({nbytes})")
    if arith not in _ARITH_DTYPES:
        raise EvcKernelError(f"unknown convolution arithmetic {arith}")
    dt = _ARITH_DTYPES[arith]
    packed = torch.empty((nbytes // dt.itemsize,), device=w.device, dtype=dt)
    _check(L.evc_conv_pack_weights(fptr(w), ptr(packed), Co, Ci, KH, KW, arith, stream_ptr()), "evc_conv_pack_weights")
    return packed


def conv_set_option(name, value):
    _check(hip_lib(require_device=False).evc_conv_set_option(name.encode(), int(value)), "evc_conv_set_option")


def packed_arith(w_packed):
    return {torch.bfloat16: ARITH_BF16X6, torch.float16: ARITH_F16X3}.get(w_packed.dtype, ARITH_F32)


_ws_cache = {}

CONV_PROFILE = None


def conv_variant(Co):
    cp = (Co + 63) // 64 * 64
    return 3 if cp % 192 == 0 else (2 if cp % 128 == 0 else 1)


def _workspace(nbytes, device):
    if torch.cuda.is_current_stream_capturing():
        return torch.empty(((nbytes + 3) // 4,), device=device, dtype=torch.float32)
    key = (device.index, torch.cuda.current_stream().cuda_stream)
    cur = _ws_cache.get(key)
    if cur is None or cur.numel() * 4 < nbytes:
        cur = torch.empty(((nbytes + 3) // 4,), device=device, dtype=torch.float32)
        _ws_cache[key] = cur
    return cur


class Cols:
    __slots__ = ("t", "c0", "C")

    def __init__(self, t, c0, C):
        assert t.is_contiguous() and 0 <= c0 and c0 + C <= t.shape[-1] and c0 % 4 == 0
        self.t, self.c0, self.C = t, c0, C


def _src(s):
    if s is None:
        return None, 0, 0, None
    if isinstance(s, Cols):
        return c_void_p(s.t.data_ptr() + 4 * s.c0), s.C, s.t.shape[-1], s.t.shape[:3]
    return ptr(s), s.shape[-1], s.shape[-1], s.shape[:3]


def conv_query_args(B, H, W, C0, C1, Co, KH, KW, arith, coef=False, act_in=ACT_NONE, splits=0, x2_ci=0, invariant=False):
    d = c_void_p(16)
    a = ConvArgs(src0=d, src1=d if C1 else None, C0=C0, C1=C1, coef_a=d if coef else None, coef_s=d if coef else None,
                 act_in=act_in, w_packed=d, out_scale=1.0, act_out=ACT_NONE, out=d, ld_out=Co, B=B, H=H, W=W, Co=Co, KH=KH,
                 KW=KW, splits=splits, arith=arith, invariant=int(bool(invariant)))
    if x2_ci:
        a.x2_src0, a.x2_C0, a.x2_w_packed, a.x2_bound = d, x2_ci, d, d
    return a


def conv_fused_1x1_supported(B, H, W, Ci, Co, arith, splits=0, invariant=False):
    a = conv_query_args(B, H, W, Ci, 0, Co, 3, 3, arith, splits=splits, invariant=invariant)
    return bool(hip_lib(require_device=False).evc_conv_fused_1x1_supported(ctypes.byref(a)))


def conv_plan(B, H, W, C0, C1, Co, K, arith, coef=False, act_in=ACT_NONE, x2_ci=0, invariant=False, splits=0):
    L = hip_lib(require_device=False)
    out = ConvPlan()
    a = conv_query_args(B, H, W, C0, C1, Co, K, K, arith, coef, act_in, splits, x2_ci, invariant)
    rc = L.evc_conv_plan_query(ctypes.byref(a), ctypes.byref(out))
    if rc != 0 and x2_ci:
        a = conv_query_args(B, H, W, C0, C1, Co, K, K, arith, coef, act_in, splits, 0, invariant)
        rc = L.evc_conv_plan_query(ctypes.byref(a), ctypes.byref(out))
    _check(rc, "evc_conv_plan_query")
    return dict(kernel=out.kernel.decode(), tile=(out.tile_m, out.tile_n), splits=out.splits,
                steps_per_split=out.steps_per_split, cut_chunk=out.cut_chunk, tail_tiles=out.tail_tiles,
                tail_splits=out.tail_splits, stats_runs=out.stats_runs, fused_1x1=bool(out.fused_1x1))


def conv_accepts(B, H, W, Ci, Co, KH, KW, arith, invariant=False):
    lib = hip_lib(require_device=False)
    a = conv_query_args(B, H, W, Ci, 0, Co, KH, KW, arith, invariant=invariant)
    return lib.evc_conv_plan_query(ctypes.byref(a), ctypes.byref(ConvPlan())) == 0 and \
        lib.evc_conv_workspace_bytes(ctypes.byref(a)) >= 0


def conv2d_nhwc(src0, w_packed, Co, KH, KW, bias=None, src1=None, coef=None, act_in=ACT_NONE, res=None,
                out_scale=1.0, act_out=ACT_NONE, out=None, splits=0, want_stats=False, in_bound=None, x2=None,
                invariant=False):
    L = hip_lib()
    inv = bool(invariant)
    p0, C0, ld0, shp = _src(src0)
    p1, C1, ld1, shp1 = _src(src1)
    assert shp1 is None or tuple(shp1) == tuple(shp)
    B, H, W = shp
    dev = (src0.t if isinstance(src0, Cols) else src0).device
    if out is None:
        out = torch.empty((B, H, W, Co), device=dev, dtype=torch.float32)
    po, Cout, ldo, shpo = _src(out)
    assert tuple(shpo) == (B, H, W) and Cout >= Co
    ca, cs = coef if coef is not None else (None, None)
    a = ConvArgs(p0, p1, C0, C1, ld0, ld1, ptr(ca), ptr(cs), act_in, ptr(w_packed), ptr(bias), ptr(res),
                 0 if res is None else res.shape[-1], float(out_scale), act_out, po, ldo,
                 B, H, W, Co, KH, KW, splits, None, packed_arith(w_packed), _word(in_bound, B if inv else 1))
    a.invariant = int(inv)
    x2_ci = 0
    if x2 is not None:
        q0, qC0, qld0, qshp = _src(x2[0])
        q1, qC1, qld1, _ = _src(x2[1])
        assert tuple(qshp) == (B, H, W) and x2[2].dtype == torch.float16
        a.x2_src0, a.x2_src1, a.x2_C0, a.x2_C1, a.x2_ld0, a.x2_ld1 = q0, q1, qC0, qC1, qld0, qld1
        a.x2_w_packed, a.x2_bound = ptr(x2[2]), _word(x2[3], B if inv else 1)
        x2_ci = qC0 + qC1
    stats = None
    if want_stats:
        ns = L.evc_conv_stats_splits(ctypes.byref(a))
        if ns > 0:
            stats = torch.empty((B, ns, Co, 2), device=dev, dtype=torch.float32)
            a.stats_out = ptr(stats)
    nbytes = L.evc_conv_workspace_bytes(ctypes.byref(a))
    if nbytes < 0:
        raise EvcKernelError(f"evc_conv_workspace_bytes rejected the arguments ({nbytes})")
    ws = _workspace(nbytes, dev) if nbytes > 0 else None
    if CONV_PROFILE is not None:
        st = torch.cuda.current_stream()
        e0, ec, e1 = (torch.cuda.Event(enable_timing=True) for _ in range(3))
        e0.record(st); ec.record(st)
        _check(L.evc_conv2d_nhwc_profiled_f32(ctypes.byref(a), ptr(ws), stream_ptr(), c_void_p(e0.cuda_event),
                                              c_void_p(ec.cuda_event)), "evc_conv2d_nhwc_profiled_f32")
        e1.record(st)
        kbuf = ctypes.create_string_buffer(96)
        L.evc_conv_kernel_name(ctypes.byref(a), kbuf, 96)
        CONV_PROFILE.append(dict(variant=conv_variant(Co), split=nbytes > 0, e0=e0, ec=ec, e1=e1, arith=a.arith,
                                 kernel=kbuf.value.decode(),
                                 flops=2.0 * B * H * W * Co * (KH * KW * (C0 + C1) + x2_ci),
                                 shape=(B, H, W, C0 + C1, Co, KH),
                                 call=dict(B=B, H=H, W=W, C0=C0, C1=C1, Co=Co, K=KH, coef=coef is not None, act_in=act_in,
                                           res=res is not None, out_scale=float(out_scale), bias=bias is not None,
                                           bound=in_bound is not None, arith=a.arith, ld_out=ldo,
                                           stats=bool(want_stats), x2=x2_ci, invariant=inv)))
    else:
        _check(L.evc_conv2d_nhwc_f32(ctypes.byref(a), ptr(ws), stream_ptr()), "evc_conv2d_nhwc_f32")
    result = out.t if isinstance(out, Cols) else out
    if want_stats:
        return result, (stats if stats is not None else chan_stats(result, invariant=inv))
    return result


def conv_fused_stats_splits(B, H, W, Ci, Co, KH, KW, splits=0, arith=None):
    a = conv_query_args(B, H, W, Ci, 0, Co, KH, KW, default_arith() if arith is None else arith, splits=splits)
    return hip_lib(require_device=False).evc_conv_stats_splits(ctypes.byref(a))


def conv_workspace_bytes(B, H, W, Ci, Co, KH, KW, splits=0, arith=None):
    a = conv_query_args(B, H, W, Ci, 0, Co, KH, KW, default_arith() if arith is None else arith, splits=splits)
    return hip_lib(require_device=False).evc_conv_workspace_bytes(ctypes.byref(a))


def attention_set_option(name, value):
    if hip_lib(require_device=False).evc_attention_set_option(name.encode(), int(value)) != 0:
        raise EvcKernelError(f"unknown attention option {name!r}")


ATTN_PROFILE = None


def attention_plan(B, heads, N, D, with_bounds=False, have_ws=None, invariant=False):
    L = hip_lib(require_device=False)
    if have_ws is None:
        nbytes = (L.evc_attention_invariant_workspace_bytes if invariant else L.evc_attention_workspace_bytes)(B, heads, N, D)
        have_ws = nbytes > 0
    out = AttentionPlan()
    _check(L.evc_attention_plan_query(B, heads, N, D, int(bool(with_bounds)), int(bool(have_ws)), int(bool(invariant)),
                                      ctypes.byref(out)), "evc_attention_plan_query")
    return dict(kernel=out.kernel.decode(), waves=out.waves, kparts=out.kparts, tiles_per_part=out.tiles_per_part,
                kv_planes=bool(out.kv_planes), merge=bool(out.merge), short_seq=bool(out.short_seq),
                lds_bytes=out.lds_bytes, parts_bytes=out.parts_bytes, ws_bytes=out.ws_bytes)


def attention(qkv, C, heads, out=None, bounds=None, invariant=False, ws=None):
    L = hip_lib()
    B, N, ld = qkv.shape
    D = C // heads
    inv = bool(invariant)
    if out is None:
        out = torch.empty((B, N, C), device=qkv.device, dtype=torch.float32)
    ld_out = out.shape[-1]
    assert out.is_contiguous() and tuple(out.shape[:2]) == (B, N) and ld_out >= C
    base = qkv.data_ptr()
    nbytes = (L.evc_attention_invariant_workspace_bytes if inv else L.evc_attention_workspace_bytes)(B, heads, N, D)
    if ws is None:
        ws = _workspace(nbytes, qkv.device) if nbytes > 0 else None
    elif ws is False:
        assert bounds is None and not inv
        ws = None
        nbytes = -1
    else:
        assert ws.dtype == torch.float32 and ws.is_contiguous() and ws.numel() * 4 >= nbytes
    if ATTN_PROFILE is not None:
        ATTN_PROFILE.append(dict(attention_plan(B, heads, N, D, bounds is not None, ws is not None, inv),
                                 call=(B, heads, N, D, bounds is not None, inv)))
    if inv:
        _check(L.evc_attention_invariant_f32(c_void_p(base), c_void_p(base + 4 * C), c_void_p(base + 8 * C), ld, fptr(out),
                                             ld_out, B, heads, N, D, float(int(D) ** (-0.5)),
                                             None if bounds is None else _word(bounds, 3 * B), ptr(ws), stream_ptr()),
               "evc_attention_invariant_f32")
        return out
    if bounds is not None:
        _check(L.evc_attention_f16x3_f32(c_void_p(base), c_void_p(base + 4 * C), c_void_p(base + 8 * C), ld, fptr(out), ld_out,
                                         B, heads, N, D, float(int(D) ** (-0.5)), _word(bounds, 3), ptr(ws), stream_ptr()),
               "evc_attention_f16x3_f32")
        return out
    if nbytes < 0:
        _check(L.evc_attention_f32(c_void_p(base), c_void_p(base + 4 * C), c_void_p(base + 8 * C), ld, fptr(out), ld_out, B,
                                   heads, N, D, float(int(D) ** (-0.5)), stream_ptr()), "evc_attention_f32")
        return out
    _check(L.evc_attention_ws_f32(c_void_p(base), c_void_p(base + 4 * C), c_void_p(base + 8 * C), ld, fptr(out), ld_out, B,
                                  heads, N, D, float(int(D) ** (-0.5)), ptr(ws), stream_ptr()), "evc_attention_ws_f32")
    return out


def frame_group_norm(x, N, gamma, beta, groups, eps):
    BN, H, W, C = x.shape
    assert BN % N == 0 and x.is_contiguous()
    y = torch.empty_like(x)
    _check(hip_lib().evc_frame_group_norm_f32(fptr(x), fptr(y), fptr(gamma), fptr(beta), BN // N, N, H * W, C, groups,
                                              float(eps), stream_ptr()), "evc_frame_group_norm_f32")
    return y


def frame_attention(qkv, N, C, heads):
    BN, H, W, ld = qkv.shape
    assert BN % N == 0 and ld == 3 * C and qkv.is_contiguous()
    out = torch.empty((BN, H, W, C), device=qkv.device, dtype=torch.float32)
    _check(hip_lib().evc_frame_attention_f32(fptr(qkv), ld, fptr(out), C, BN // N, N, H * W, C, heads,
                                             float(int(C // heads) ** (-0.5)), stream_ptr()), "evc_frame_attention_f32")
    return out


def frame_mix(x, N, w, bias):
    BN, H, W, C = x.shape
    M = w.shape[0]
    assert BN % N == 0 and tuple(w.shape) == (M, N) and x.is_contiguous() and w.is_contiguous()
    B = BN // N
    y = torch.empty((B * M, H, W, C), device=x.device, dtype=torch.float32)
    _check(hip_lib().evc_frame_mix_f32(fptr(x), fptr(y), fptr(w), fptr(bias), B, N, M, H * W * C, stream_ptr()),
           "evc_frame_mix_f32")
    return y


def frame_taps(x, N):
    BN, H, W, C = x.shape
    assert BN % N == 0 and x.is_contiguous()
    y = torch.empty((BN, H, W, 3 * C), device=x.device, dtype=torch.float32)
    _check(hip_lib().evc_frame_taps_f32(fptr(x), fptr(y), BN // N, N, H * W, C, stream_ptr()), "evc_frame_taps_f32")
    return y


class Deconv5x5s2:

    def __init__(self, weight, bias, arith=None, device="cuda"):
        Lh = hip_lib()
        w = weight.detach().to(device, torch.float32).contiguous()
        self.Ci, self.Co = w.shape[0], w.shape[1]
        self.Cp, self.CiPad = (self.Co + 15) // 16 * 16, (self.Ci + 15) // 16 * 16
        wp = torch.empty((4 * self.Cp, self.CiPad, 3, 3), device=device, dtype=torch.float32)
        _check(Lh.evc_deconv5x5s2_phase_weights_f32(fptr(w), fptr(wp), self.Ci, self.Co, self.Cp, self.CiPad, stream_ptr()),
               "evc_deconv5x5s2_phase_weights_f32")
        self.arith = default_arith() if arith is None else arith
        self.w = conv_pack_weights(wp, self.arith)
        b4 = torch.zeros((4, self.Cp), device=device, dtype=torch.float32)
        b4[:, :self.Co] = bias.detach().to(device, torch.float32)[None, :]
        self.bias4 = b4.reshape(-1).contiguous()

    def __call__(self, x, act_out=ACT_NONE):
        B, H, W, C = x.shape
        assert C == self.CiPad and x.dtype == torch.float32 and x.is_contiguous()
        Lh = hip_lib()
        ws = _workspace(Lh.evc_deconv5x5s2_workspace_bytes(B, H, W, self.Cp), x.device)
        out = torch.empty((B, 2 * H, 2 * W, self.Co), device=x.device, dtype=torch.float32)
        _check(Lh.evc_deconv5x5s2_f32(fptr(x), ptr(self.w), self.arith, fptr(self.bias4), fptr(out), ptr(ws), B, H, W, C,
                                      self.Co, act_out, stream_ptr()), "evc_deconv5x5s2_f32")
        return out


class Conv5x5s2:

    def __init__(self, weight, bias, arith=None, device="cuda"):
        Lh = hip_lib()
        w = weight.detach().to(device, torch.float32).contiguous()
        self.Co, self.Ci = w.shape[0], w.shape[1]
        self.Cq = (self.Ci + 3) // 4 * 4
        wq = torch.empty((self.Co, 4 * self.Cq, 3, 3), device=device, dtype=torch.float32)
        _check(Lh.evc_conv5x5s2_phase_weights_f32(fptr(w), fptr(wq), self.Co, self.Ci, self.Cq, stream_ptr()),
               "evc_conv5x5s2_phase_weights_f32")
        self.arith = default_arith() if arith is None else arith
        self.w = conv_pack_weights(wq, self.arith)
        self.bias = bias.detach().to(device, torch.float32).contiguous()

    def __call__(self, x, act_out=ACT_NONE, channels=None):
        B, H2, W2, ld = x.shape
# ... 386 lines not shown
```

### extreme-video-compression-with-prediction-using-pre-trainded-diffusion-models-_amd/scorenet.py

```python
import math
from types import SimpleNamespace

import numpy as np
import torch

from . import lib as L

FIR_K = np.outer([1, 3, 3, 1], [1, 3, 3, 1]).astype(np.float32)
FIR_K /= FIR_K.sum()
INV_SQRT2 = float(np.float32(1.0) / np.sqrt(np.float32(2.0)))


def num_groups(ch):
    g = min(ch // 4, 32)
    while ch % g != 0:
        g -= 1
    return g


def dims_from_config(config):
    m, d = config.model, config.data
    return SimpleNamespace(ngf=m.ngf, ch_mult=list(m.ch_mult), num_res_blocks=m.num_res_blocks,
                           attn_resolutions=list(m.attn_resolutions), n_head_channels=m.n_head_channels,
                           image_size=d.image_size, channels=d.channels, num_frames=d.num_frames,
# ... 41 lines not shown
def range_sites(program, cond_emb=False):
    sites = []
    for i, m in enumerate(program):
        n = f"all_modules.{i + (1 if cond_emb and i >= 2 else 0)}"
        k = m["kind"]
        if k == "res":
            has_skip = m["cin"] != m["cout"] or m["up"] or m["down"]
            sites.append(dict(tag="res0", module=i, name=n + ".Conv_0", consumers=[(i, "w0")]))
            sites.append(dict(tag="res1", module=i, name=n + ".Conv_1", consumers=[(i, "w1")] + ([(i, "w2")] if has_skip else [])))
        elif k == "attn":
            sites.append(dict(tag="attn_norm", module=i, name=n + ".NIN_0-2", consumers=[(i, "wqkv")]))
            sites.append(dict(tag="attn_qkv", module=i, name=n + ".NIN_3", consumers=[(i, "attention"), (i, "wo")]))
        elif k == "norm":
            sites.append(dict(tag="norm", module=i, name=f"all_modules.{i + 1 + (1 if cond_emb else 0)}",
                              consumers=[(i + 1, "w")]))
    for j, st in enumerate(sites):
        st["site"] = j
    return sites


class _Act:
    __slots__ = ("t", "_stats", "invariant")

    def __init__(self, t, stats=None, invariant=False):
        self.t = t
        self._stats = stats
        self.invariant = invariant

    def stats(self):
        if self._stats is None:
            self._stats = L.chan_stats(self.t, invariant=self.invariant)
        return self._stats


def _f16_only(w_packed, bound):
    return bound if L.packed_arith(w_packed) == L.ARITH_F16X3 else None


def _pad16(c):
    return (c + 15) // 16 * 16


class DdpmWrapper:

    def _init_wrapper(self, m, sigma_begin, sigma_end, num_classes):
        self.noise_in_cond = bool(getattr(m, "noise_in_cond", False))
        self.cond_noise_fn = None
        self.cond_generator = None
        dist = getattr(m, "sigma_dist", "linear")
        if dist == "linear":
            self.betas = torch.linspace(sigma_begin, sigma_end, num_classes)
            self.alphas = torch.cumprod(1 - self.betas.flip(0), 0).flip(0)
            self.alphas_prev = torch.cat([self.alphas[1:], torch.tensor([1.0]).to(self.alphas)])
        elif dist == "cosine":
            T = num_classes
            t = torch.linspace(T, 0, T + 1) / T
            f = torch.cos((t + 0.008) / (1 + 0.008) * math.pi / 2) ** 2
            self.alphas = f[:-1] / f[-1]
            self.alphas_prev = torch.cat([self.alphas[1:], torch.tensor([1.0]).to(self.alphas)])
            self.betas = 1 - self.alphas / self.alphas_prev
        else:
            raise NotImplementedError(f"sigma_dist {dist!r}: the reference builds its buffers for 'linear' and 'cosine' only")
        self.gamma = bool(getattr(m, "gamma", False))
        if self.gamma:
            self.theta_0 = 0.001
            self.k = self.betas / (self.alphas * (self.theta_0 ** 2))
            self.k_cum = torch.cumsum(self.k.flip(0), 0).flip(0)
            self.theta_t = torch.sqrt(self.alphas) * self.theta_0

    def _noised_cond(self, cond, vals):
        if not self.noise_in_cond or cond is None:
            return cond
        if any(v != int(v) or v < 0 for v in vals):
            raise IndexError("noise_in_cond indexes the schedule with the labels (alphas[labels]): integer labels only")
        raw = None if self.cond_noise_fn is None else self.cond_noise_fn(cond).to(self.device, torch.float32).contiguous()
        out = torch.empty_like(cond)
        start = 0
        while start < len(vals):
            end = start
            while end < len(vals) and vals[end] == vals[start]:
                end += 1
            i = int(vals[start])
            a = self.alphas[i]
            c = cond[start:end].contiguous()
            if self.gamma:
                from .sampler import _gamma_noise
                z = _gamma_noise(c, self.k_cum[i], self.theta_t[i], a, raw=None if raw is None else raw[start:end],
                                 generator=self.cond_generator)
            elif raw is not None:
                z = raw[start:end].contiguous()
            else:
                z = torch.randn(c.shape, device=self.device, dtype=torch.float32, generator=self.cond_generator)
            out[start:end] = L.lincomb4([c, z], [float(a.sqrt()), float((1 - a).sqrt())])
            start = end
        return out


class ScoreNet(DdpmWrapper):

    SPADE = False
    ARCH = "unetmore"
    RANGE_SITES = True

    def __init__(self, config, state_dict, device="cuda", prefix="", preactivate=False, use_graphs=False, demote=(),
                 batch_invariant=False):
        self.batch_invariant = bool(batch_invariant)
        if self.batch_invariant and (self.SPADE or self.ARCH != "unetmore"):
            raise NotImplementedError("batch_invariant is built for the concat-conditioned score network (ScoreNet) only")
        if self.batch_invariant and demote:
            raise ValueError("batch-invariant mode does not combine with demoted sites (range recovery): a receiver could not "
                             "know which layers the sender demoted")
        L.hip_lib()
        self.preactivate = preactivate
        self.config = config
        self.device = torch.device(device)
        self.d = dims_from_config(config)
        self.type = getattr(config.model, "type", "v1")
        m = config.model
        if bool(getattr(m, "spade", False)) != self.SPADE or getattr(m, "output_all_frames", False) or m.arch != self.ARCH:
            raise NotImplementedError("built: arch=unetmore -- the concat-conditioned network of configs/mine.yml (ScoreNet) and its "
                                      "SPADE variant (SpadeScoreNet) -- and arch=unetmorepseudo3d / unetmore3d without SPADE "
                                      "(Pseudo3dScoreNet / Conv3dScoreNet), all without output_all_frames (which fails in the "
                                      "reference itself: ncsnpp_more.py:384-385 splits 15 channels into 6 + 15)")
        self.cond_emb = bool(getattr(m, "cond_emb", False))
        self._init_wrapper(m, self.d.sigma_begin, self.d.sigma_end, self.d.num_classes)
        if self.batch_invariant and self.noise_in_cond:
            raise NotImplementedError("batch_invariant with noise_in_cond: the conditioning noise is drawn per batch")
        if (self.cond_emb or self.noise_in_cond) and self.SPADE:
            raise NotImplementedError("cond_emb / noise_in_cond are built for the concat-conditioned network only")
        self.embed_dim = self._embed_dim()
        self.program = self._build_program()
        if self.SPADE:
            self.program[2]["cin"] = self.d.channels * self.d.num_frames
        self._wsrc = {}
        self._load(state_dict, prefix + "unet.all_modules.")
        self.sites = range_sites(self.program, self.cond_emb) if self.RANGE_SITES else []
        self.site_words = L.site_word_arena(len(self.sites), self.device)
        self._demoted = set()
        self._attn_f32 = set()
        self._unfused = set()
        self._site_of = {}
        self._set_site_args()
        self.demote_seconds = 0.0
        self._rows = {}
        self._row_tensors = {}
        self._table = torch.zeros((256, self.ss_total), device=self.device, dtype=torch.float32)
        self._n_rows = 0
        self.use_graphs = use_graphs
        self._graphs = {}
        self._f16_raw = L.bounded_arith() == L.ARITH_F16X3
        import os
        self.overlap_skip = os.environ.get("EVC_OVERLAP_SKIP", "1") != "0"
        self.fuse_skip = self._f16_raw and os.environ.get("EVC_FUSE_SKIP", "1") != "0"
        self._side_streams = {}
        self._bounds_by_stream = {}
        self._bounds = None
        self._bound_next = 0
        self._bound_batch = 1
        if demote:
            self.demote(demote)

    def _conv(self, *a, **kw):
        return L.conv2d_nhwc(*a, invariant=self.batch_invariant, **kw)

    def _act(self, t, stats=None):
        return _Act(t, stats, invariant=self.batch_invariant)

    def _gn(self, *a, **kw):
        return L.gn_coeffs(*a, invariant=self.batch_invariant, **kw)

    def _mbound(self, *a, **kw):
        return L.moments_bound(*a, invariant=self.batch_invariant, **kw)

    def _attention(self, *a, **kw):
        return L.attention(*a, invariant=self.batch_invariant, **kw)

    def _fuse_ok(self, *a, **kw):
        return L.conv_fused_1x1_supported(*a, invariant=self.batch_invariant, **kw)

    def invariant_view(self):
        import copy
        if self.batch_invariant:
            return self
        if self.SPADE or self.ARCH != "unetmore" or self.noise_in_cond:
            raise NotImplementedError("batch_invariant is built for the concat-conditioned score network (ScoreNet) only")
        if self._demoted:
            raise ValueError("batch-invariant mode does not combine with demoted sites (range recovery)")
        v = copy.copy(self)
        v.batch_invariant = True
        v.taps = None
        v._rows, v._row_tensors = {}, {}
        v._table = torch.zeros_like(self._table)
        v._n_rows = 0
        v._graphs, v._side_streams, v._bounds_by_stream = {}, {}, {}
        v._bounds, v._bound_next = None, 0
        return v

    def _set_site_args(self):
        self._site_of = {(st["tag"], st["module"]): L.Site(self.site_words, st["site"], quiet=st["site"] in self._demoted)
                         for st in self.sites}

    def _site(self, tag, i):
        return self._site_of.get((tag, i))

    def _site_ids(self, sites):
        by_name = {st["name"]: st["site"] for st in self.sites}
        out = []
        for s in sites:
            k = by_name.get(s) if isinstance(s, str) else int(s)
            if k is None or not 0 <= k < len(self.sites):
                raise KeyError(f"no range-event site {s!r} in this network")
            out.append(k)
        return out

    def demote(self, sites):
        import time
        if self.batch_invariant:
            raise ValueError("batch-invariant mode does not combine with demoted sites (range recovery)")
        new = [k for k in dict.fromkeys(self._site_ids(sites)) if k not in self._demoted]
        if not new:
            return []
        t0 = time.perf_counter()
        for k in new:
            for i, key in self.sites[k]["consumers"]:
                if key == "attention":
                    self._attn_f32.add(i)
                    continue
                if key in ("w1", "w2"):
                    self._unfused.add(i)
                if L.packed_arith(self.w[i][key]) == L.ARITH_F16X3:
                    w, pad_ci = self._wsrc[(i, key)]
                    self.w[i][key] = self._repack(w, pad_ci, L.ARITH_BF16X6)
            self._demoted.add(k)
        self._set_site_args()
        self._graphs.clear()
        torch.cuda.synchronize(self.device)
        self.demote_seconds += time.perf_counter() - t0
        return new

    def demoted_sites(self):
        return {k: self.sites[k]["name"] for k in sorted(self._demoted)}

    def _build_program(self):
        return build_program(self.d)

    def _embed_dim(self):
        return self.d.ngf

    def _dev(self, t):
        return t.detach().to(device=self.device, dtype=torch.float32).contiguous()

    def _pack_conv(self, w, pad_ci=None, bounded=False):
        return self._repack(w, pad_ci, L.bounded_arith() if bounded else L.default_arith())

    def _repack(self, w, pad_ci, arith):
        w = self._dev(w)
        if pad_ci is not None and pad_ci != w.shape[1]:
            wp = torch.zeros((w.shape[0], pad_ci, w.shape[2], w.shape[3]), device=self.device)
            wp[:, :w.shape[1]] = w
            w = wp
        return L.conv_pack_weights(w, arith)

    def _pack_site(self, i, key, w, pad_ci=None):
        self._wsrc[(i, key)] = (w, pad_ci)
        return self._pack_conv(w, pad_ci, bounded=True)

    def _load(self, sd, pre):
        g = lambda name: sd[name]
        self.w = {}
        dense_w, dense_b = [], []
        off = 0
        if self.cond_emb:
            self.cond_table = self._dev(g(pre + "2.weight"))
            assert tuple(self.cond_table.shape) == (2, self.d.ngf // 2), tuple(self.cond_table.shape)
        for i, m in enumerate(self.program):
            n = pre + str(i + (1 if self.cond_emb and i >= 2 else 0))
            k = m["kind"]
            if k == "linear":
                w = g(n + ".weight")
                self.w[i] = dict(w=self._pack_conv(w[:, :, None, None]), b=self._dev(g(n + ".bias")),
                                 co=w.shape[0])
            elif k in ("conv_in", "conv_out"):
                w = g(n + ".weight")
                self.w[i] = dict(w=(self._pack_site(i, "w", w, _pad16(w.shape[1])) if k == "conv_out" else
                                    self._pack_conv(w, _pad16(w.shape[1]))),
                                 b=self._dev(g(n + ".bias")),
                                 co=w.shape[0], cin_pad=_pad16(w.shape[1]))
            elif k == "res":
                e = dict()
                for j, key in ((0, "actnorm0"), (1, "actnorm1")):
                    dw, db = g(f"{n}.{key}.Dense_0.weight"), g(f"{n}.{key}.Dense_0.bias")
                    dense_w.append(dw); dense_b.append(db)
                    e[f"ss{j}"] = (off, dw.shape[0] // 2)
                    off += dw.shape[0]
                    self._load_actnorm(e, j, f"{n}.{key}", g)
                e["w0"] = self._pack_site(i, "w0", g(n + ".Conv_0.weight")); e["b0"] = self._dev(g(n + ".Conv_0.bias"))
                e["w1"] = self._pack_site(i, "w1", g(n + ".Conv_1.weight")); e["b1"] = self._dev(g(n + ".Conv_1.bias"))
                if m["cin"] != m["cout"] or m["up"] or m["down"]:
                    e["w2"] = self._pack_site(i, "w2", g(n + ".Conv_2.weight")); e["b2"] = self._dev(g(n + ".Conv_2.bias"))
                    e["b12"] = (e["b1"] + e["b2"]).contiguous()
                self.w[i] = e
            elif k == "attn":
                ws = [g(f"{n}.NIN_{j}.W") for j in range(4)]
                bs = [g(f"{n}.NIN_{j}.b") for j in range(4)]
                wqkv = torch.cat([w.t() for w in ws[:3]], 0)[:, :, None, None]
                self.w[i] = dict(gamma=self._dev(g(n + ".GroupNorm_0.weight")),
# ... 13 lines not shown

    def _load_final_norm(self, n, g):
        return dict(gamma=self._dev(g(n + ".Norm_0.weight")), beta=self._dev(g(n + ".Norm_0.bias")))

    def _embedding(self, labels):
        dim = self.embed_dim
        half = dim // 2
        emb = math.log(10000) / (half - 1)
        emb = torch.exp(torch.arange(half, dtype=torch.float32) * -emb)
        emb = torch.tensor(labels, dtype=torch.float32)[:, None] * emb[None, :]
        return torch.cat([torch.sin(emb), torch.cos(emb)], dim=1)

    def _key(self, label, mask=1):
        return (float(label), int(mask)) if self.cond_emb else float(label)

    def prepare_labels(self, labels, masks=None):
        masks = [1] * len(labels) if masks is None else masks
        new = [k for k in dict.fromkeys(self._key(x, mk) for x, mk in zip(labels, masks)) if k not in self._rows]
        if not new:
            return
        R = len(new)
        if self.batch_invariant:
            return self._prepare_rows(new, (R, 1, 1))
        return self._prepare_rows(new, (1, 1, R))

    def _prepare_rows(self, new, shape):
        R = len(new)
        e = self._embedding([k[0] if self.cond_emb else k for k in new]).to(self.device).reshape(*shape, self.embed_dim).contiguous()
        w0, w1 = self.w[0], self.w[1]
        t = self._conv(e, w0["w"], w0["co"], 1, 1, bias=w0["b"])
        t = self._conv(t, w1["w"], w1["co"], 1, 1, bias=w1["b"], act_in=L.ACT_SILU)
        if self.cond_emb:
            emb = self.cond_table[torch.tensor([k[1] for k in new], device=self.device)]
            t = torch.cat([t.reshape(R, -1), emb], 1).reshape(*shape, -1).contiguous()
        rows = self._conv(t, self.dense_w, self.ss_total, 1, 1, bias=self.dense_b, act_in=L.ACT_SILU)
        base = self._n_rows
        if base + R > self._table.shape[0]:
            grown = torch.zeros((max(2 * self._table.shape[0], base + R), self.ss_total), device=self.device)
            grown[:base] = self._table[:base]
            self._table = grown
            self._graphs.clear()
        self._table[base:base + R] = rows.reshape(R, self.ss_total)
        self._n_rows = base + R
        for j, v in enumerate(new):
            self._rows[v] = base + j

    def _row_tensor(self, row_ids):
        key = tuple(row_ids)
        t = self._row_tensors.get(key)
        if t is None:
            t = torch.tensor(row_ids, dtype=torch.int32, device=self.device)
            self._row_tensors[key] = t
        return t

    def _adagn(self, parts, hw, ch, seg, rows, bound=None, site=None):
        off, c = seg
        assert c == ch
        return self._gn(parts, hw, num_groups(ch), 1e-5, mode=2, ss=self._table[:, off:off + 2 * c], row=rows,
                           bound=bound, site=site)

    def _side_stream(self, main):
        key = main.cuda_stream
        st = self._side_streams.get(key)
        if st is None:
            st = self._side_streams[key] = torch.cuda.Stream(device=self.device)
        return st

    def _bound_slot(self, n=1):
        if not self._f16_raw:
            return None
        n *= self._bound_batch
        w = self._bounds[self._bound_next:self._bound_next + n]
        self._bound_next += n
        return w

    def _res(self, i, m, x, skip, rows):
        e = self.w[i]
        B, H, W, _ = x.t.shape
        parts = [x.stats()] + ([skip.stats()] if skip is not None else [])
        xbound = self._bound_slot() if "w2" in e else None
        coef0 = self._adagn(parts, H * W, m["cin"], e["ss0"], rows, bound=xbound, site=self._site("res0", i))
        fir = None
        if m["up"] or m["down"]:
            fir = (FIR_K * 4.0, 2, 1, (2, 1)) if m["up"] else (FIR_K, 1, 2, (1, 1))
        s1 = None if skip is None else skip.t

        def skip_path(out):
            src, src1 = x.t, s1
            if fir is not None:
                src, src1 = L.upfirdn2d_nhwc(x.t, *fir), None
            if "w2" in e:
                return self._conv(src, e["w2"], m["cout"], 1, 1, bias=e["b2"], src1=src1, in_bound=_f16_only(e["w2"], xbound),
                                     out=out)
            return src

        Ho, Wo = (2 * H, 2 * W) if m["up"] else ((H // 2, W // 2) if m["down"] else (H, W))
        fuse = self.fuse_skip and "w2" in e and not self.preactivate and i not in self._unfused and \
            self._fuse_ok(B, Ho, Wo, m["cout"], m["cout"], L.packed_arith(e["w1"]))
        side = done = xs = None
        if self.overlap_skip and "w2" in e and (not fuse or fir is not None):
            main = torch.cuda.current_stream()
            side = self._side_stream(main)
            xs = torch.empty((B, Ho, Wo, m["cin"] if fuse else m["cout"]), device=self.device, dtype=torch.float32)
            side.wait_stream(main)
            with torch.cuda.stream(side):
                if fuse:
                    L.upfirdn2d_nhwc(x.t, *fir, out=xs)
                else:
                    skip_path(xs)
                done = torch.cuda.Event()
                done.record(side)
        if fir is not None:
            hf = L.upfirdn2d_nhwc(x.t, *fir, coef=coef0, act=L.ACT_SILU)
            h1 = self._act(*self._conv(hf, e["w0"], m["cout"], 3, 3, bias=e["b0"], want_stats=True))
        elif self.preactivate:
            cin = m["cin"]
            act = torch.empty((B, H, W, cin), device=self.device, dtype=torch.float32)
            c0 = x.t.shape[3]
            L.affine_act(x.t, coef0, L.ACT_SILU, out=L.Cols(act, 0, c0))
            if skip is not None:
                L.affine_act(skip.t, coef0, L.ACT_SILU, out=L.Cols(act, c0, cin - c0), coef_col=c0)
            h1 = self._act(*self._conv(act, e["w0"], m["cout"], 3, 3, bias=e["b0"], want_stats=True))
        else:
            h1 = self._act(*self._conv(x.t, e["w0"], m["cout"], 3, 3, bias=e["b0"], src1=s1, coef=coef0, act_in=L.ACT_SILU,
                                     want_stats=True))
        H1, W1 = h1.t.shape[1], h1.t.shape[2]
        coef1 = self._adagn([h1.stats()], H1 * W1, m["cout"], e["ss1"], rows, site=self._site("res1", i))
        if side is None:
            if fuse:
                xs = L.upfirdn2d_nhwc(x.t, *fir) if fir is not None else None
            else:
                xs = skip_path(None)
        else:
            torch.cuda.current_stream().wait_event(done)
        if fuse:
            x2 = (xs, None, e["w2"], xbound) if xs is not None else (x.t, s1, e["w2"], xbound)
            return self._act(*self._conv(h1.t, e["w1"], m["cout"], 3, 3, bias=e["b12"], coef=coef1, act_in=L.ACT_SILU,
                                       out_scale=INV_SQRT2, want_stats=True, x2=x2))
        if self.preactivate:
            h1a = L.affine_act(h1.t, coef1, L.ACT_SILU)
            return self._act(*self._conv(h1a, e["w1"], m["cout"], 3, 3, bias=e["b1"], res=xs, out_scale=INV_SQRT2,
                                       want_stats=True))
        return self._act(*self._conv(h1.t, e["w1"], m["cout"], 3, 3, bias=e["b1"], coef=coef1, act_in=L.ACT_SILU,
                                   res=xs, out_scale=INV_SQRT2, want_stats=True))

    def _attn(self, i, m, x):
        e = self.w[i]
        B, H, W, C = x.t.shape
        hd = self.d.n_head_channels
        heads = 1 if C < hd else C // hd
        coef = self._gn([x.stats()], H * W, num_groups(C), 1e-6, mode=1, gamma=e["gamma"], beta=e["beta"],
                           site=self._site("attn_norm", i))
        qkvb = self._bound_slot(3)
        if qkvb is None:
            obound = None
            qkv = self._conv(x.t, e["wqkv"], 3 * C, 1, 1, bias=e["bqkv"], coef=coef)
        else:
            qkv, qst = self._conv(x.t, e["wqkv"], 3 * C, 1, 1, bias=e["bqkv"], coef=coef, want_stats=True)
            self._mbound(qst, 0, C, qkvb, site=self._site("attn_qkv", i))
            obound = _f16_only(e["wo"], qkvb.view(B, 3)[:, 2].contiguous() if self.batch_invariant else qkvb[2:3])
        o = self._attention(qkv.view(B, H * W, 3 * C), C, heads, bounds=None if i in self._attn_f32 else qkvb)
        return self._act(*self._conv(o.view(B, H, W, C), e["wo"], C, 1, 1, bias=e["bo"], res=x.t,
                                   out_scale=INV_SQRT2, want_stats=True, in_bound=obound))

    @torch.no_grad()
    def forward_rows(self, x, rows, cond=None):
        if self.batch_invariant and self._demoted:
            raise ValueError("batch-invariant mode does not combine with demoted sites (range recovery)")
        return self._forward_rows(x, rows, cond)

    def _forward_rows(self, x, rows, cond=None):
        d = self.d
        prog = self.program
        B, _, H, W = x.shape
        self._bound_batch = B if self.batch_invariant else 1
        nb = 256 * self._bound_batch
        if self._f16_raw:
            if torch.cuda.is_current_stream_capturing():
                self._bounds = torch.empty(nb, device=self.device, dtype=torch.int32)
            else:
                key = torch.cuda.current_stream().cuda_stream
                self._bounds = self._bounds_by_stream.get(key)
                if self._bounds is None or self._bounds.numel() != nb:
                    self._bounds = self._bounds_by_stream[key] = torch.empty(nb, device=self.device, dtype=torch.int32)
            self._bounds.zero_()
            self._bound_next = 0
        taps = getattr(self, "taps", None)

        def tap(idx, act):
            if taps is not None:
                taps[idx] = act.t[..., :prog[idx].get("cout", prog[idx].get("ch"))].permute(0, 3, 1, 2).contiguous()
            return act
        i = 2
        m = prog[i]
        xin = self._pack_input(x, cond, self.w[i]["cin_pad"])
        hs = [tap(i, self._act(*self._conv(xin, self.w[i]["w"], m["cout"], 3, 3, bias=self.w[i]["b"], want_stats=True)))]
        i += 1
        n_lvl = len(d.ch_mult)
        for lvl in range(n_lvl):
            for _ in range(d.num_res_blocks):
                h = tap(i, self._res(i, prog[i], hs[-1], None, rows)); i += 1
                if h.t.shape[2] in d.attn_resolutions:
                    h = tap(i, self._attn(i, prog[i], h)); i += 1
                hs.append(h)
            if lvl != n_lvl - 1:
                hs.append(tap(i, self._res(i, prog[i], hs[-1], None, rows))); i += 1
        h = hs[-1]
        h = tap(i, self._res(i, prog[i], h, None, rows)); i += 1
        h = tap(i, self._attn(i, prog[i], h)); i += 1
        h = tap(i, self._res(i, prog[i], h, None, rows)); i += 1
        for lvl in reversed(range(n_lvl)):
            for _ in range(d.num_res_blocks + 1):
                h = tap(i, self._res(i, prog[i], h, hs.pop(), rows)); i += 1
            if h.t.shape[2] in d.attn_resolutions:
                h = tap(i, self._attn(i, prog[i], h)); i += 1
            if lvl != 0:
                h = tap(i, self._res(i, prog[i], h, None, rows)); i += 1
        assert not hs
        out, co = self._final(i, h)
        assert i + 2 == len(prog)
        res = L.nhwc_to_nchw(out, co)
        if taps is not None:
            taps[i + 1] = res
        return res

    def _pack_input(self, x, cond, cin_pad):
        return L.pack_nchw_to_nhwc(x, cond, cin_pad)

    def _final(self, i, h):
        e = self.w[i]
        B, H, W, C = h.t.shape
        coef = self._gn([h.stats()], H * W, num_groups(C), 1e-5, mode=1, gamma=e["gamma"], beta=e["beta"],
                           site=self._site("norm", i))
        co = self.program[i + 1]["cout"]
        out = torch.empty((B, H, W, _pad16(co)), device=h.t.device, dtype=torch.float32)
        self._conv(h.t, self.w[i + 1]["w"], co, 3, 3, bias=self.w[i + 1]["b"], coef=coef, act_in=L.ACT_SILU, out=out)
        return out, co

    def _forward(self, x, rows, cond):
        if not self.use_graphs:
            return self.forward_rows(x, rows, cond)
        key = (torch.cuda.current_stream().cuda_stream, tuple(x.shape), cond is not None, self.preactivate)
        g = self._graphs.get(key)
        if g is None:
            g = self._capture(x, rows, cond)
            self._graphs[key] = g
        g["x"].copy_(x)
        g["rows"].copy_(rows)
        if cond is not None:
            g["cond"].copy_(cond)
        g["graph"].replay()
        return g["out"].clone()

    def _capture(self, x, rows, cond):
        sx, srows = x.clone(), rows.clone()
        scond = None if cond is None else cond.clone()
        cur = torch.cuda.current_stream()
        side = torch.cuda.Stream(device=self.device)
        side.wait_stream(cur)
        with torch.cuda.stream(side):
            self.forward_rows(sx, srows, scond)
        cur.wait_stream(side)
        torch.cuda.synchronize(self.device)
        graph = torch.cuda.CUDAGraph()
        with torch.cuda.graph(graph):
            out = self.forward_rows(sx, srows, scond)
        return dict(graph=graph, x=sx, rows=srows, cond=scond, out=out)

    def forward_label(self, x, label, cond=None):
        self.prepare_labels([label])
        rows = self._row_tensor([self._rows[self._key(label)]] * x.shape[0])
        if self.noise_in_cond and cond is not None:
            cond = self._noised_cond(cond.to(self.device, torch.float32).contiguous(), [float(label)] * x.shape[0])
        return self._forward(x, rows, cond)

    def __call__(self, x, labels, cond=None, cond_mask=None):
        vals = [float(v) for v in (labels.detach().cpu().tolist() if torch.is_tensor(labels) else labels)]
        assert len(vals) == x.shape[0]
        masks = None
        if self.cond_emb and cond_mask is not None:
            masks = [int(v) for v in (cond_mask.detach().cpu().tolist() if torch.is_tensor(cond_mask) else cond_mask)]
        self.prepare_labels(vals, masks)
        rows = self._row_tensor([self._rows[self._key(v, 1 if masks is None else masks[j])] for j, v in enumerate(vals)])
        x = x.to(self.device, torch.float32).contiguous()
        cond = None if cond is None else cond.to(self.device, torch.float32).contiguous()
        return self._forward(x, rows, self._noised_cond(cond, vals))

    forward = __call__

    def eval(self):
        return self


def build_score_network(config, state_dict, device="cuda", **kw):
    arch = getattr(config.model, "arch", "unetmore")
    if arch == "unet":
        from .unet_ddpm import UNetDDPM
        return UNetDDPM(config, state_dict, device=device, batch_invariant=kw.get("batch_invariant", False))
    if arch in ("unetmorepseudo3d", "unetmore3d"):
        from .scorenet_pseudo3d import Conv3dScoreNet, Pseudo3dScoreNet
        return (Conv3dScoreNet if arch == "unetmore3d" else Pseudo3dScoreNet)(config, state_dict, device=device, **kw)
    if getattr(config.model, "spade", False):
        from .scorenet_spade import SpadeScoreNet
        return SpadeScoreNet(config, state_dict, device=device, **kw)
    return ScoreNet(config, state_dict, device=device, **kw)
```

### include/evc_hip.h

```cpp
#ifndef EVC_HIP_H
#define EVC_HIP_H

#ifdef __cplusplus
extern "C" {
#endif

#define EVC_OK 0
#define EVC_EINVAL (-1)
#define EVC_EUNSUPPORTED (-2)
#define EVC_ELAUNCH (-3)

#define EVC_ACT_NONE 0
#define EVC_ACT_SILU 1
#define EVC_ACT_RELU 2

#define EVC_ARITH_F32 0
#define EVC_ARITH_BF16X6 1
#define EVC_ARITH_F16X3 2

const char* evc_version(void);
const char* evc_arch(void);
int evc_device_ok(void);

int evc_clock_probe(unsigned long long* out2, int spin_us, const unsigned* stop, void* stream);

int evc_upfirdn2d_f32(const float* input, float* out, const float* kernel_host, int major, int in_h, int in_w,
                      int kh, int kw, int up_x, int up_y, int down_x, int down_y, int pad_x0, int pad_x1,
                      int pad_y0, int pad_y1, void* stream);

int evc_upfirdn2d_nhwc_f32(const float* x, float* out, const float* kernel_host, int B, int H, int W, int C,
                           int kh, int kw, int up, int down, int pad0, int pad1, const float* coef_a,
                           const float* coef_s, int act, void* stream);

int evc_pack_nchw_to_nhwc_f32(const float* x0, int C0, const float* x1, int C1, float* out, int Cpad, int B,
                              int H, int W, void* stream);
int evc_nhwc_to_nchw_f32(const float* in, int ld, float* out, int B, int C, int H, int W, void* stream);

int evc_chan_stats_f32(const float* x, float* partial, int B, int HW, int C, int nsplit, void* stream);

int evc_gn_coeffs_f32(const float* part0, int nsplit0, int C0, const float* part1, int nsplit1, int C1, int B,
                      int HW, int groups, float eps, int mode, const float* gamma, const float* beta,
                      const float* ss, int ss_ld, const int* row, float* coef_a, float* coef_s, void* stream);

#define EVC_RANGE_NONFINITE 1u
#define EVC_RANGE_F16_OPERAND 2u

int evc_gn_coeffs_bound_f32(const float* part0, int nsplit0, int C0, const float* part1, int nsplit1, int C1, int B,
                            int HW, int groups, float eps, int mode, const float* gamma, const float* beta,
                            const float* ss, int ss_ld, const int* row, float* coef_a, float* coef_s,
                            unsigned* bound_bits, unsigned* events, void* stream);
int evc_moments_bound_f32(const float* part, int nsplit, int C, int c_begin, int c_count, int n_ranges, int B,
                          unsigned* bound_bits, unsigned* events, void* stream);

int evc_gn_coeffs_site_f32(const float* part0, int nsplit0, int C0, const float* part1, int nsplit1, int C1, int B,
                           int HW, int groups, float eps, int mode, const float* gamma, const float* beta,
                           const float* ss, int ss_ld, const int* row, float* coef_a, float* coef_s, unsigned* events,
                           unsigned* site_events, int site, void* stream);
int evc_gn_coeffs_bound_site_f32(const float* part0, int nsplit0, int C0, const float* part1, int nsplit1, int C1, int B,
                                 int HW, int groups, float eps, int mode, const float* gamma, const float* beta,
                                 const float* ss, int ss_ld, const int* row, float* coef_a, float* coef_s,
                                 unsigned* bound_bits, unsigned* events, unsigned* site_events, int site, void* stream);
int evc_moments_bound_site_f32(const float* part, int nsplit, int C, int c_begin, int c_count, int n_ranges, int B,
                               unsigned* bound_bits, unsigned* events, unsigned* site_events, int site, void* stream);

int evc_affine_act_nhwc_f32(const float* x, float* y, const float* coef_a, const float* coef_s, int act, int B,
                            int HW, int C, int ld_coef, int ld_out, void* stream);

int evc_spade_act_nhwc_f32(const float* x, float* y, const float* coef_a, const float* coef_s, int ld_coef,
                           const float* gmap, const float* bmap, int ld_map, const float* ss_scale,
                           const float* ss_shift, int ld_ss, const int* row, int act, int B, int HW, int C, int ld_out,
                           void* stream);

typedef struct {
    const float* src0; const float* src1; int C0; int C1;
    int ld0; int ld1;
    const float* coef_a; const float* coef_s; int act_in;
    const float* w_packed; const float* bias; const float* res; int ld_res;
    float out_scale; int act_out;
    float* out; int ld_out;
    int B; int H; int W; int Co; int KH; int KW;
    int splits;
    float* stats_out;
    int arith;
    const unsigned* in_bound;
    const float* x2_src0; const float* x2_src1; int x2_C0; int x2_C1; int x2_ld0; int x2_ld1;
    const float* x2_w_packed; const unsigned* x2_bound;
    int invariant;
} evc_conv_args;
int evc_conv_co_pad(int Co);
long long evc_conv_packed_floats(int Co, int Ci, int KH, int KW);
int evc_conv_pack_weights_f32(const float* w, float* packed, int Co, int Ci, int KH, int KW, void* stream);
long long evc_conv_packed_bytes(int Co, int Ci, int KH, int KW, int arith);
int evc_conv_pack_weights(const float* w, void* packed, int Co, int Ci, int KH, int KW, int arith, void* stream);
int evc_conv_set_option(const char* name, int value);
int evc_conv_kernel_name(const evc_conv_args* a, char* buf, int n);
int evc_conv_choose_splits(const evc_conv_args* a);
int evc_conv_fused_1x1_supported(const evc_conv_args* a);
int evc_conv_stats_splits(const evc_conv_args* a);
long long evc_conv_workspace_bytes(const evc_conv_args* a);
int evc_conv2d_nhwc_f32(const evc_conv_args* a, float* ws, void* stream);

#define EVC_INVARIANT_REF_BATCH 9
int evc_invariant_plan_revision(void);
typedef struct {
    char kernel[96];
    int tile_m, tile_n, splits, steps_per_split, cut_chunk, tail_tiles, tail_splits, stats_runs, fused_1x1;
} evc_conv_plan;
int evc_conv_plan_query(const evc_conv_args* a, evc_conv_plan* out);
int evc_gn_coeffs_bound_sample_f32(const float* part0, int nsplit0, int C0, const float* part1, int nsplit1, int C1, int B,
                                   int HW, int groups, float eps, int mode, const float* gamma, const float* beta,
                                   const float* ss, int ss_ld, const int* row, float* coef_a, float* coef_s,
                                   unsigned* bound_bits, unsigned* events, unsigned* site_events, int site, void* stream);
int evc_moments_bound_sample_f32(const float* part, int nsplit, int C, int c_begin, int c_count, int n_ranges, int B,
                                 unsigned* bound_bits, unsigned* events, unsigned* site_events, int site, void* stream);
long long evc_attention_invariant_workspace_bytes(int B, int heads, int N, int D);
int evc_attention_invariant_f32(const float* q, const float* k, const float* v, int ld_qkv, float* out, int ld_out, int B,
                                int heads, int N, int D, float scale, const unsigned* bounds, float* ws, void* stream);

int evc_conv2d_nhwc_profiled_f32(const evc_conv_args* a, float* ws, void* stream, void* ev_start, void* ev_conv_end);

int evc_attention_f32(const float* q, const float* k, const float* v, int ld_qkv, float* out, int ld_out, int B,
                      int heads, int N, int D, float scale, void* stream);
long long evc_attention_workspace_bytes(int B, int heads, int N, int D);
int evc_attention_set_option(const char* name, int value);
int evc_attention_ws_f32(const float* q, const float* k, const float* v, int ld_qkv, float* out, int ld_out, int B,
                         int heads, int N, int D, float scale, float* ws, void* stream);

int evc_attention_f16x3_f32(const float* q, const float* k, const float* v, int ld_qkv, float* out, int ld_out, int B,
                            int heads, int N, int D, float scale, const unsigned* bounds, float* ws, void* stream);

typedef struct {
    char kernel[64];
    int waves, kparts, tiles_per_part, kv_planes, merge, short_seq;
    long long lds_bytes, parts_bytes, ws_bytes;
} evc_attention_plan;
int evc_attention_plan_query(int B, int heads, int N, int D, int with_bounds, int have_ws, int invariant,
                             evc_attention_plan* out);

int evc_frame_group_norm_f32(const float* x, float* y, const float* gamma, const float* beta, int B, int N, int HW, int C,
                             int groups, float eps, void* stream);
int evc_frame_attention_f32(const float* qkv, int ld_qkv, float* out, int ld_out, int B, int N, int HW, int C, int heads,
                            float scale, void* stream);
int evc_frame_mix_f32(const float* x, float* y, const float* w, const float* bias, int B, int N, int M, long long inner,
                      void* stream);

int evc_frame_taps_f32(const float* x, float* y, int B, int N, int HW, int C, void* stream);

int evc_ddpm_step_f32(float* x, const float* e, const float* noise, long long n, float k1, float k2, float c1,
                      float c2, float sigma, int clip, void* stream);
int evc_ddim_step_f32(float* x, const float* e, long long n, float k1, float k2, float c1, float c2, int clip,
                      void* stream);
int evc_axpy_f32(const float* x, const float* e, float* y, long long n, float alpha, void* stream);
int evc_pndm_transfer_f32(const float* x, const float* e, float* y, long long n, float d, float cx, float ce,
                          int clip, void* stream);
int evc_lincomb4_f32(const float* e0, const float* e1, const float* e2, const float* e3, float* y, long long n,
                     float w0, float w1, float w2, float w3, void* stream);
int evc_scale_clamp_f32(const float* x, float* y, long long n, float mul, float add, int clamp, float lo, float hi,
                        void* stream);

int evc_gate_residual_f32(const float* a, const float* b, const float* x, float* out, long long n, void* stream);
int evc_elic_gather_params_f32(const float* ms, int ld, int mean_off, int scale_off, int C, int B, int H, int W,
                               int parity, const float* scale_table, int n_scales, int* idx, float* means,
                               void* stream);
int evc_elic_scatter_symbols_f32(const int* symbols, const float* means, float* y_hat, int ld, int c0, int C,
                                 int B, int H, int W, int parity, void* stream);
int evc_elic_quantize_f32(const float* y, int ld, int c0, const float* means, int C, int B, int H, int W,
                          int parity, int* symbols, void* stream);

int evc_elic_rate_pass_f32(const float* ms, int ld, int mean_off, int scale_off, int C, const float* y, int ld_y, int c0,
                           int B, int H, int W, int parity, float* y_hat, double* bits, void* stream);
int evc_bottleneck_rate_f32(const float* z, int ld, int C, int B, int H, int W, const float* medians, const float* density,
                            float* z_hat, double* bits, void* stream);

int evc_deconv5x5s2_phase_weights_f32(const float* wt, float* wp, int Ci, int Co, int Cp, int CiPad, void* stream);
int evc_conv5x5s2_phase_weights_f32(const float* w, float* wq, int Co, int Ci, int Cq, void* stream);
int evc_depth_to_space2_f32(const float* in, int ld_in, int Cp, float* out, int C, int B, int H, int W, void* stream);
int evc_space_to_depth2_f32(const float* in, int ld_in, int C, float* out, int ld_out, int Cq, int B, int H, int W,
                            void* stream);
long long evc_deconv5x5s2_workspace_bytes(int B, int H, int W, int Cp);
int evc_deconv5x5s2_f32(const float* x, const void* w_packed, int arith, const float* bias4, float* out, float* ws, int B,
                        int H, int W, int Ci, int Co, int act_out, void* stream);
long long evc_conv5x5s2_workspace_bytes(int B, int Ho, int Wo, int Ci);
int evc_conv5x5s2_f32(const float* x, int ld_in, const void* w_packed, int arith, const float* bias, float* out, float* ws,
                      int B, int Ho, int Wo, int Ci, int Co, int act_out, void* stream);

int evc_im2col_nchw_f32(const float* x, float* out, int N, int C, int H, int W, int KH, int KW, int stride, int pad, int ld_out,
                        const float* shift, const float* scale, void* stream);
int evc_maxpool3s2_nhwc_f32(const float* x, float* out, int N, int H, int W, int C, void* stream);
int evc_lpips_layer_f32(const float* f0, const float* f1, const float* lin_w, float* dist, int N, int HW, int C, int accumulate,
                        void* stream);

int evc_maxpool2d_nhwc_f32(const float* x, float* out, int N, int H, int W, int C, int k, int stride, int ceil_mode, void* stream);
int evc_lpips_map_f32(const float* f0, const float* f1, const float* lin_w, float* map, int N, int HW, int C, void* stream);
int evc_lpips_map_mean_f32(const float* map, float* dist, int N, int HW, int accumulate, void* stream);
int evc_lpips_upsample_add_f32(const float* map, float* out, int N, int h, int w, int H, int W, int accumulate, void* stream);

int evc_i3d_stem_im2col_f32(const float* x, float* out, int B, int T, int C, int H, int W, int Hr, int Wr, int R, int KT, int KH,
                            int KW, int ST, int SH, int SW, int f_begin, int nf, int ld_out, void* stream);
int evc_maxpool3d_same_nthwc_f32(const float* x, float* out, int B, int T, int H, int W, int C, int KT, int KH, int KW, int ST,
                                 int SH, int SW, void* stream);
int evc_i3d_head_f32(const float* x, const float* w, const float* bias, float* out, int B, int T, int HW, int C, int Co, int KT,
                     void* stream);

long long evc_gdn_workspace_bytes(int B, int H, int W, int C);
int evc_gdn_f32(const float* x, const void* gamma_packed, int arith, const float* beta, float* out, float* ws, int B,
                int H, int W, int C, int inverse, int simplified, void* stream);

int evc_noise_normal_f32(float* out, const unsigned* keys, int B, long long n, unsigned long long seed, unsigned step,
                         int raw, void* stream);

#define EVC_YUV_NEAREST 0
#define EVC_YUV_BILINEAR 1
#define EVC_YUV_BICUBIC 2
int evc_yuv420_to_rgb(const unsigned char* src, long long src_bytes, long long first, long long frame_stride, long long off_y,
                      long long off_u, long long off_v, int N, int H, int W, int bits, int mode, void* out, int out_u8,
                      void* stream);
int evc_rgb_to_yuv420(const float* rgb, unsigned char* dst, long long dst_bytes, long long first, long long frame_stride,
                      long long off_y, long long off_u, long long off_v, int N, int H, int W, int bits, unsigned* events,
                      void* stream);

int evc_resample_h_u8(const unsigned char* src, int planes, int rows, int cols, long long plane_stride, long long row_stride,
                      const int* bounds, const int* coeffs, int ksize, int n_out, unsigned char* dst, void* stream);
int evc_resample_v_u8(const unsigned char* src, int planes, int rows, int cols, long long plane_stride, long long row_stride,
                      const int* bounds, const int* coeffs, int ksize, int n_out, unsigned char* dst, void* stream);

int evc_tile_grid_check(int N, int H, int W, int S, int ny, int nx, const int* oy_host, const int* ox_host, int cover);
int evc_tile_gather_u8(const unsigned char* src, int N, int H, int W, int S, int ny, int nx, const int* oy_host,
                       const int* ox_host, const int* oy, const int* ox, unsigned char* dst, void* stream);
int evc_tile_blend_f32(const float* tiles, int N, int H, int W, int S, int ny, int nx, const int* oy_host, const int* ox_host,
                       const int* oy, const int* ox, float* out, void* stream);

long long evc_ssim_workspace_bytes(int N, int H, int W);
int evc_ssim_planes_f32(const float* a, const float* b, int N, int H, int W, const double* taps11, double c1, double c2,
                        double* out, void* ws, void* stream);

#define EVC_POOL_AVG 0
#define EVC_POOL_MAX 1
int evc_inception_stem_im2col_f32(const float* x, float* out, int N, int C, int H, int W, int f_begin, int nf, int ld_out,
                                  void* stream);
int evc_im2col_nhwc_f32(const float* x, float* out, int N, int H, int W, int C, int KH, int KW, int SH, int SW, int PH, int PW,
                        int ld_out, void* stream);
int evc_pool3x3s1p1_nhwc_f32(const float* x, float* out, int N, int H, int W, int C, int mode, void* stream);
int evc_spatial_mean_nhwc_f32(const float* x, float* out, int N, int HW, int C, void* stream);
int evc_knn_radius_f32(const float* x, double* radius2, int n, int d, int k, void* stream);
int evc_manifold_hits_f32(const float* y, const float* x, const double* radius2, int* flags, int m, int n, int d, void* stream);

#ifdef __cplusplus
}
#endif
#endif
```

Baseline: 37.49.

## Add dedicated f16-split 1x1 projection GEMM kernel for attention qkv and output

Adds a specialized GEMM kernel for 1x1 projections in attention blocks. It uses f16 two-term split MFMA, keeps the weight chunks in registers across several steps, and fuses the bias, residual, scaling, per-tile statistics and range-bound atomics into the epilogue. For the qkv projection this removes the separate stats pass and bound-reduction launch. The scorenet uses it by default for the f16 raw path whenever the shape is supported and the generic conv plan would not already pick a single-split 128-row tile. Shared split arithmetic moves into a common header.

Result: no change. 37.84 (median of 6 runs) (+0.9%).

```diff
diff --git a/extreme-video-compression-with-prediction-using-pre-trainded-diffusion-models-_amd/build.py b/extreme-video-compression-with-prediction-using-pre-trainded-diffusion-models-_amd/build.py
--- a/extreme-video-compression-with-prediction-using-pre-trainded-diffusion-models-_amd/build.py
+++ b/extreme-video-compression-with-prediction-using-pre-trainded-diffusion-models-_amd/build.py
@@ -9,7 +9,7 @@
 LIBDIR = os.path.join(HERE, "lib")
 OBJDIR = os.path.join(HERE, "build")
 INCLUDE = os.path.join(os.path.dirname(HERE), "include")
-HIP_SOURCES = ["conv_igemm.hip", "attention.hip", "norm.hip", "fir.hip", "elementwise.hip", "gdn.hip", "stride2.hip", "lpips.hip", "i3d.hip", "frames.hip", "noise.hip", "yuv.hip", "rate.hip", "ssim.hip", "inception.hip", "resample.hip", "tile.hip", "api.hip"]
+HIP_SOURCES = ["conv_igemm.hip", "proj_gemm.hip", "attention.hip", "norm.hip", "fir.hip", "elementwise.hip", "gdn.hip", "stride2.hip", "lpips.hip", "i3d.hip", "frames.hip", "noise.hip", "yuv.hip", "rate.hip", "ssim.hip", "inception.hip", "resample.hip", "tile.hip", "api.hip"]
 ARCH = "gfx950"
 
 
@@ -37,6 +37,7 @@
     os.makedirs(LIBDIR, exist_ok=True)
     os.makedirs(OBJDIR, exist_ok=True)
     headers = [os.path.join(INCLUDE, h) for h in ("evc_hip.h", "evc_rans.h")]
+    headers += [os.path.join(CSRC, h) for h in sorted(os.listdir(CSRC)) if h.endswith(".h")]
     hipcc = hipcc_path()
     flags = ["--offload-arch=" + ARCH, "-O3", "-std=c++17", "-fPIC", "-I", INCLUDE]
     flags += os.environ.get("EVC_HIPCC_FLAGS", "").split()
diff --git a/extreme-video-compression-with-prediction-using-pre-trainded-diffusion-models-_amd/csrc/conv_igemm.hip b/extreme-video-compression-with-prediction-using-pre-trainded-diffusion-models-_amd/csrc/conv_igemm.hip
--- a/extreme-video-compression-with-prediction-using-pre-trainded-diffusion-models-_amd/csrc/conv_igemm.hip
+++ b/extreme-video-compression-with-prediction-using-pre-trainded-diffusion-models-_amd/csrc/conv_igemm.hip
@@ -2,8 +2,8 @@
 #include <stdint.h>
 #include <stdio.h>
 #include "../../include/evc_hip.h"
-
-typedef float f32x16 __attribute__((ext_vector_type(16)));
+#include "split_arith.h"
+
 typedef __attribute__((address_space(3))) void lds_void;
 typedef const __attribute__((address_space(1))) void glb_void;
 
@@ -24,62 +24,10 @@
 namespace {
 
 constexpr int BM_MAX = 128;
-constexpr int KC = 16;
-
-constexpr int MODE_PLAIN = 0, MODE_AFFINE = 1, MODE_AFFINE_SILU = 2, MODE_SILU = 3, MODE_RELU = 4;
-
-struct ConvK {
-    const float* src0; const float* src1; int C0; int C1; int ld0; int ld1;
-    const float* coef_a; const float* coef_s;
-    const float* w; const float* bias; const float* res; int ld_res;
-    float out_scale; int act_out;
-    float* out; int ld_out;
-    int B, H, W, Co, CoPad, KH, KW;
-    int M, HW, nchunk, nsteps, steps_per_split, splits;
-    float* ws;
-    float* stats;
-    const float* w_hdr;
-    const unsigned* in_bound;
-    int tail_first, tail_splits, tail_sps, tail_rows;
-    int cut_chunk;
-    const float* x2_src0; const float* x2_src1; int x2_C0, x2_C1, x2_ld0, x2_ld1;
-    const char* x2_w;
-    const float* x2_hdr;
-    const unsigned* x2_bound;
-    int bound_stride, generic_epi;
-};
-
-__device__ __forceinline__ float bound_scale(unsigned bits) {
-    const float b = sqrtf(__uint_as_float(bits));
-    if (!(b < 3.0e38f)) return __builtin_nanf("");
-    return b > 0.f ? ldexpf(1.0f, 6 - ilogbf(b)) : 1.0f;
-}
-__device__ __forceinline__ int bound_index(const ConvK& p, int m) { return p.bound_stride ? min(m, p.M - 1) / p.HW : 0; }
-__device__ __forceinline__ float in_scale(const ConvK& p, int m) {
-    if (!p.in_bound) return 1.0f;
-    return bound_scale(p.in_bound[bound_index(p, m)]);
-}
-
-__device__ __forceinline__ float silu_f(float v) { return v * __builtin_amdgcn_rcpf(1.0f + __expf(-v)); }
 
 __device__ __forceinline__ float act_fn(float v, int act) {
     if (act == EVC_ACT_SILU) return silu_f(v);
     if (act == EVC_ACT_RELU) return v < 0.f ? 0.f : v;
-    return v;
-}
-
-template <int MODE>
-__device__ __forceinline__ float4 transform(float4 v, const float4& a, const float4& s, bool ok) {
-    if (MODE == MODE_AFFINE || MODE == MODE_AFFINE_SILU) {
-        v.x = v.x * a.x + s.x; v.y = v.y * a.y + s.y; v.z = v.z * a.z + s.z; v.w = v.w * a.w + s.w;
-    }
-    if (MODE == MODE_AFFINE_SILU || MODE == MODE_SILU) {
-        v.x = silu_f(v.x); v.y = silu_f(v.y); v.z = silu_f(v.z); v.w = silu_f(v.w);
-    }
-    if (MODE == MODE_RELU) {
-        v.x = v.x < 0.f ? 0.f : v.x; v.y = v.y < 0.f ? 0.f : v.y; v.z = v.z < 0.f ? 0.f : v.z; v.w = v.w < 0.f ? 0.f : v.w;
-    }
-    v.x = ok ? v.x : 0.f; v.y = ok ? v.y : 0.f; v.z = ok ? v.z : 0.f; v.w = ok ? v.w : 0.f;
     return v;
 }
 
@@ -348,57 +296,6 @@
     conv_epilogue<TM, TN>(p, acc, m0, n0, split, wm, wn, l31, half);
 }
 
-typedef __bf16 bf16x8 __attribute__((ext_vector_type(8)));
-typedef _Float16 f16x8 __attribute__((ext_vector_type(8)));
-
-__device__ __forceinline__ void split3_bf16(const float4& v0, const float4& v1, bf16x8& p1, bf16x8& p2, bf16x8& p3) {
-    const float x[8] = {v0.x, v0.y, v0.z, v0.w, v1.x, v1.y, v1.z, v1.w};
-#pragma unroll
-    for (int j = 0; j < 8; ++j) {
-        const __bf16 a = (__bf16)x[j];
-        const float r = x[j] - (float)a;
-        const __bf16 b = (__bf16)r;
-        p1[j] = a; p2[j] = b; p3[j] = (__bf16)(r - (float)b);
-    }
-}
-
-constexpr float F16_ACT_SCALE = 8.0f;
-
-__device__ __forceinline__ void split2_f16(const float4& v0, const float4& v1, float xscale, f16x8& p1, f16x8& p2) {
-    const float x[8] = {v0.x, v0.y, v0.z, v0.w, v1.x, v1.y, v1.z, v1.w};
-#pragma unroll
-    for (int j = 0; j < 8; ++j) {
-        const float v = x[j] * xscale;
-        const _Float16 a = (_Float16)v;
-        p1[j] = a; p2[j] = (_Float16)(v - (float)a);
-    }
-}
-
-template <int NP> struct Split;
-template <> struct Split<3> {
-    typedef bf16x8 vec;
-    static constexpr int NTERM = 6;
-    static __device__ __forceinline__ constexpr int qa(int t) { return t == 0 ? 2 : (t == 1 || t == 3) ? 1 : 0; }
-    static __device__ __forceinline__ constexpr int qb(int t) { return t == 2 ? 2 : (t == 1 || t == 4) ? 1 : 0; }
-    static __device__ __forceinline__ f32x16 mfma(const vec& a, const vec& b, const f32x16& c) {
-        return __builtin_amdgcn_mfma_f32_32x32x16_bf16(a, b, c, 0, 0, 0);
-    }
-    static __device__ __forceinline__ void split(const float4& v0, const float4& v1, float, vec (&pl)[3]) {
-        split3_bf16(v0, v1, pl[0], pl[1], pl[2]);
-    }
-};
-template <> struct Split<2> {
-    typedef f16x8 vec;
-    static constexpr int NTERM = 3;
-    static __device__ __forceinline__ constexpr int qa(int t) { return t == 0 ? 1 : 0; }
-    static __device__ __forceinline__ constexpr int qb(int t) { return t == 1 ? 1 : 0; }
-    static __device__ __forceinline__ f32x16 mfma(const vec& a, const vec& b, const f32x16& c) {
-        return __builtin_amdgcn_mfma_f32_32x32x16_f16(a, b, c, 0, 0, 0);
-    }
-    static __device__ __forceinline__ void split(const float4& v0, const float4& v1, float xscale, vec (&pl)[2]) {
-        split2_f16(v0, v1, xscale, pl[0], pl[1]);
-    }
-};
 
 template <int NP, int TM, int TN, int MODE>
 __global__ __launch_bounds__(256, 2) void conv_splitn_kernel(ConvK p) {
@@ -781,7 +678,6 @@
 
     conv_epilogue<TM, TN>(p, acc, m0, n0, split, wm, wn, l31, half);
 }
-
 
 template <int NP, int WM, int TN, int MODE>
 __global__ __launch_bounds__(128 * WM, WM == 2 ? 2 : 1) void conv_split_rr_kernel(ConvK p) {
@@ -1641,8 +1537,6 @@
     }
 }
 
-constexpr int F16_HDR_BYTES = 256;
-
 __global__ void conv_absmax_kernel(const float* w, size_t n, unsigned* out_bits) {
     float m = 0.f;
     for (size_t i = (size_t)blockIdx.x * blockDim.x + threadIdx.x; i < n; i += (size_t)gridDim.x * blockDim.x)
diff --git a/extreme-video-compression-with-prediction-using-pre-trainded-diffusion-models-_amd/csrc/proj_gemm.hip b/extreme-video-compression-with-prediction-using-pre-trainded-diffusion-models-_amd/csrc/proj_gemm.hip
--- /dev/null
+++ b/extreme-video-compression-with-prediction-using-pre-trainded-diffusion-models-_amd/csrc/proj_gemm.hip
@@ -0,0 +1,290 @@
+#include <hip/hip_runtime.h>
+#include <stdint.h>
+#include <type_traits>
+#include "../../include/evc_hip.h"
+#include "split_arith.h"
+
+namespace {
+
+constexpr int PG_BM = 64;
+constexpr int PG_G = 4;
+constexpr int PG_RB = 32;
+constexpr int PG_PLANE = PG_BM * PG_RB;
+constexpr int PG_CHUNK = 2 * PG_PLANE + 256;
+constexpr int PG_BUF = PG_G * PG_CHUNK;
+constexpr unsigned PG_NAN_BITS = 0x7fc00000u;
+
+struct ProjK {
+    ConvK c;
+    unsigned* bound_bits;
+    int n_ranges, range_c;
+    unsigned* events;
+    unsigned* site_events;
+};
+
+__device__ __forceinline__ constexpr int pg_chunk_base(int q) { return q * PG_CHUNK + 16 * (q & 1) + 128 * (q >> 1); }
+
+__device__ __forceinline__ void pg_raise_word(unsigned* w, unsigned bits) {
+    if (w && (__hip_atomic_load(w, __ATOMIC_RELAXED, __HIP_MEMORY_SCOPE_AGENT) & bits) != bits) atomicOr(w, bits);
+}
+
+template <int MODE>
+__global__ __launch_bounds__(256, 2) void proj_gemm_kernel(ProjK pk) {
+    typedef Split<2> SP;
+    typedef f16x8 vec;
+    constexpr int TN = 1, BN = 64 * TN;
+    constexpr int DEPTH = 2;
+    constexpr bool HAS_COEF = MODE == MODE_AFFINE;
+    const ConvK& p = pk.c;
+    extern __shared__ __attribute__((aligned(16))) char pg_smem[];
+    char* const As = pg_smem;
+    float* const coef_l = reinterpret_cast<float*>(pg_smem + 2 * PG_BUF);
+
+    const int tid = threadIdx.x;
+    const int lane = tid & 63;
+    const int wave = __builtin_amdgcn_readfirstlane(tid >> 6);
+    const int wm = wave >> 1, wn = wave & 1;
+    const int l31 = lane & 31, half = lane >> 5;
+    const int m0 = blockIdx.x * PG_BM;
+    const int n0 = blockIdx.y * BN;
+    const int C = p.C0;
+    const int nchunk = p.nchunk;
+    const int nsteps = (nchunk + PG_G - 1) / PG_G;
+
+    const int row = tid >> 2, q = tid & 3;
+    const float* const xrow = p.src0 + (size_t)(m0 + row) * p.ld0;
+    const int a_lds0 = pg_chunk_base(q) + row * PG_RB + 16 * (0 ^ ((row >> 3) & 1));
+    const int a_lds1 = pg_chunk_base(q) + row * PG_RB + 16 * (1 ^ ((row >> 3) & 1));
+    const float xscale = F16_ACT_SCALE * in_scale(p, m0);
+    float4 xr[4];
+    int a_c = 0;
+    auto load_a = [&](int s) {
+        a_c = min(PG_G * s + q, nchunk - 1);
+        const float4* src = reinterpret_cast<const float4*>(xrow + a_c * KC);
+#pragma unroll
+        for (int i = 0; i < 4; ++i) xr[i] = src[i];
+    };
+    auto store_a = [&](int buf) {
+        float4 ca[4], cs[4];
+        if (HAS_COEF) {
+#pragma unroll
+            for (int i = 0; i < 4; ++i) {
+                ca[i] = *reinterpret_cast<const float4*>(coef_l + a_c * KC + 4 * i);
+                cs[i] = *reinterpret_cast<const float4*>(coef_l + C + a_c * KC + 4 * i);
+            }
+        }
+        char* A = As + buf * PG_BUF;
+#pragma unroll
+        for (int kh = 0; kh < 2; ++kh) {
+            vec pl[2];
+            SP::split(transform<MODE>(xr[2 * kh], ca[2 * kh], cs[2 * kh], true),
+                      transform<MODE>(xr[2 * kh + 1], ca[2 * kh + 1], cs[2 * kh + 1], true), xscale, pl);
+            char* d = A + (kh ? a_lds1 : a_lds0);
+            *reinterpret_cast<vec*>(d) = pl[0];
+            *reinterpret_cast<vec*>(d + PG_PLANE) = pl[1];
+        }
+    };
+
+    const unsigned planeB = (unsigned)p.CoPad * PG_RB;
+    const unsigned slab = 2u * planeB;
+    const unsigned wlane = (unsigned)(n0 + wn * 32 * TN + l31) * PG_RB + 16u * (unsigned)(half ^ ((l31 >> 3) & 1));
+    const char* const wbase = reinterpret_cast<const char*>(p.w);
+    vec b[DEPTH][PG_G][TN][2];
+    auto load_b = [&](int set, int c, int s) {
+        const char* wt = wbase + (unsigned)min(PG_G * s + c, nchunk - 1) * slab + wlane;
+#pragma unroll
+        for (int j = 0; j < TN; ++j) {
+            b[set][c][j][0] = *reinterpret_cast<const vec*>(wt + j * 32 * PG_RB);
+            b[set][c][j][1] = *reinterpret_cast<const vec*>(wt + planeB + j * 32 * PG_RB);
+        }
+    };
+    const int a_rd = (wm * 32 + l31) * PG_RB + 16 * (half ^ ((l31 >> 3) & 1));
+
+    f32x16 acc[TN];
+#pragma unroll
+    for (int j = 0; j < TN; ++j)
+#pragma unroll
+        for (int r = 0; r < 16; ++r) acc[j][r] = 0.f;
+
+    load_a(0);
+#pragma unroll
+    for (int d = 0; d < DEPTH; ++d)
+#pragma unroll
+        for (int c = 0; c < PG_G; ++c) load_b(d, c, d);
+    if (HAS_COEF) {
+        const int bimg = m0 / p.HW;
+        const float4* ga = reinterpret_cast<const float4*>(p.coef_a + (size_t)bimg * C);
+        const float4* gs = reinterpret_cast<const float4*>(p.coef_s + (size_t)bimg * C);
+        for (int i = tid; i < (C >> 2); i += 256) {
+            reinterpret_cast<float4*>(coef_l)[i] = ga[i];
+            reinterpret_cast<float4*>(coef_l + C)[i] = gs[i];
+        }
+        __syncthreads();
+    }
+    store_a(0);
+    if (nsteps > 1) load_a(1);
+    __syncthreads();
+
+    auto super_step = [&](int s, auto set, auto inner) {
+        constexpr int SET = decltype(set)::value;
+        constexpr bool INNER = decltype(inner)::value;
+        const int buf = s & 1;
+#pragma unroll
+        for (int c = 0; c < PG_G; ++c) {
+            if (INNER || PG_G * s + c < nchunk) {
+                const char* Ab = As + buf * PG_BUF + pg_chunk_base(c) + a_rd;
+                vec a[2];
+                a[0] = *reinterpret_cast<const vec*>(Ab);
+                a[1] = *reinterpret_cast<const vec*>(Ab + PG_PLANE);
+#pragma unroll
+                for (int t = 0; t < SP::NTERM; ++t)
+#pragma unroll
+                    for (int j = 0; j < TN; ++j) acc[j] = SP::mfma(a[SP::qa(t)], b[SET][c][j][SP::qb(t)], acc[j]);
+            }
+            if (INNER) {
+                load_b(SET, c, s + DEPTH);
+                if (c == 1) {
+                    store_a(buf ^ 1);
+                    if (s + 2 < nsteps) load_a(s + 2);
+                }
+            }
+        }
+        __syncthreads();
+    };
+    typedef std::integral_constant<int, 0> set0;
+    typedef std::integral_constant<int, 1> set1;
+    int s = 0;
+    for (; s + 2 < nsteps; s += 2) {
+        super_step(s, set0(), std::true_type());
+        super_step(s + 1, set1(), std::true_type());
+    }
+    if (s + 2 == nsteps) { super_step(s, set0(), std::true_type()); ++s; }
+    if ((s & 1) == 0) super_step(s, set0(), std::false_type());
+    else super_step(s, set1(), std::false_type());
+
+    const float ascale = p.w_hdr[0] / in_scale(p, m0);
+    const float oscale = p.out_scale;
+    const int mw = m0 + wm * 32 + 4 * half;
+    const int cw = n0 + wn * 32 * TN + l31;
+    const bool moments = p.stats != nullptr || pk.bound_bits != nullptr;
+    float ssum[TN], ssq[TN];
+#pragma unroll
+    for (int j = 0; j < TN; ++j) {
+        const int co = cw + j * 32;
+        const float bias = p.bias ? p.bias[co] : 0.f;
+        float rv[16];
+#pragma unroll
+        for (int r = 0; r < 16; ++r) rv[r] = 0.f;
+        if (p.res) {
+            const float* rp = p.res + (size_t)mw * p.ld_res + co;
+#pragma unroll
+            for (int r = 0; r < 16; ++r) rv[r] = rp[(size_t)((r & 3) + 8 * (r >> 2)) * p.ld_res];
+        }
+        float* o = p.out + (size_t)mw * p.ld_out + co;
+        float st_sum = 0.f, st_sq = 0.f;
+#pragma unroll
+        for (int r = 0; r < 16; ++r) {
+            const float v = (acc[j][r] * ascale + bias + rv[r]) * oscale;
+            o[(size_t)((r & 3) + 8 * (r >> 2)) * p.ld_out] = v;
+            st_sum += v; st_sq += v * v;
+        }
+        ssum[j] = st_sum + __shfl_xor(st_sum, 32);
+        ssq[j] = st_sq + __shfl_xor(st_sq, 32);
+    }
+    if (!moments) return;
+    float2* const sc = reinterpret_cast<float2*>(pg_smem);
+    if (wm == 1 && half == 0) {
+#pragma unroll
+        for (int j = 0; j < TN; ++j) sc[(wn * TN + j) * 32 + l31] = make_float2(ssum[j], ssq[j]);
+    }
+    __syncthreads();
+    if (wm == 1) return;
+    float mx = 0.f;
+    unsigned bad = 0;
+    int zcur = -1;
+    auto flush = [&]() {
+        if (zcur < 0) return;
+#pragma unroll
+        for (int off = 16; off > 0; off >>= 1) mx = fmaxf(mx, __shfl_xor(mx, off));
+        const bool anybad = __any(bad) != 0;
+        if (lane == 0) {
+            const unsigned bits = anybad ? PG_NAN_BITS : __float_as_uint(mx);
+            unsigned* const word = pk.bound_bits + zcur;
+            if (bits > __hip_atomic_load(word, __ATOMIC_RELAXED, __HIP_MEMORY_SCOPE_AGENT)) atomicMax(word, bits);
+            if (anybad) { pg_raise_word(pk.events, EVC_RANGE_NONFINITE); pg_raise_word(pk.site_events, EVC_RANGE_NONFINITE); }
+        }
+        mx = 0.f; bad = 0;
+    };
+#pragma unroll
+    for (int j = 0; j < TN; ++j) {
+        const float2 e = sc[(wn * TN + j) * 32 + l31];
+        const float sum = ssum[j] + e.x, sq = ssq[j] + e.y;
+        const int co = cw + j * 32;
+        if (p.stats && half == 0) {
+            float* sp = p.stats + ((size_t)(m0 / PG_BM) * p.Co + co) * 2;
+            sp[0] = sum; sp[1] = sq;
+        }
+        if (pk.bound_bits) {
+            const int z = (n0 + wn * 32 * TN + j * 32) / pk.range_c;
+            if (z != zcur) { flush(); zcur = z; }
+            mx = fmaxf(mx, sq);
+            bad |= !(fabsf(sum) < 3.0e38f) | !(sq < 3.0e38f);
+        }
+    }
+    if (pk.bound_bits) flush();
+}
+
+constexpr long long PG_LDS_CAP = 64 * 1024;
+
+int proj_validate(const evc_proj_args* a) {
+    if (!a || !a->x || !a->w_packed || !a->out) return EVC_EINVAL;
+    if (a->B <= 0 || a->HW <= 0 || a->C <= 0 || a->Co <= 0 || a->C1 < 0) return EVC_EINVAL;
+    if (a->C1 > 0 && !a->x1) return EVC_EINVAL;
+    if ((a->coef_a == nullptr) != (a->coef_s == nullptr)) return EVC_EINVAL;
+    if (a->ld_x != 0 && (a->ld_x < a->C || (a->ld_x & 3))) return EVC_EINVAL;
+    if (a->ld_out < a->Co || (a->res && a->ld_res < a->Co)) return EVC_EINVAL;
+    if ((long long)a->B * a->HW > 0x7fffffffLL) return EVC_EINVAL;
+    if (a->arith != EVC_ARITH_F32 && a->arith != EVC_ARITH_BF16X6 && a->arith != EVC_ARITH_F16X3) return EVC_EINVAL;
+    if (a->n_ranges < 0 || (a->n_ranges > 0) != (a->bound_bits != nullptr)) return EVC_EINVAL;
+    if (a->site_events && a->site < 0) return EVC_EINVAL;
+    if (((uintptr_t)a->x | (uintptr_t)a->coef_a | (uintptr_t)a->coef_s | (uintptr_t)a->w_packed) & 15) return EVC_EINVAL;
+    if (a->arith != EVC_ARITH_F16X3 || a->C1 > 0 || a->x1) return EVC_EUNSUPPORTED;
+    if (a->C % KC != 0 || a->Co % 192 != 0 || a->HW % PG_BM != 0) return EVC_EUNSUPPORTED;
+    if (a->n_ranges > 0 && (a->Co % a->n_ranges != 0 || (a->Co / a->n_ranges) % 32 != 0)) return EVC_EUNSUPPORTED;
+    if (4LL * a->C * evc_conv_co_pad(a->Co) > 0x7fffffffLL) return EVC_EUNSUPPORTED;
+    if (2LL * PG_BUF + (a->coef_a ? 8LL * a->C : 0) > PG_LDS_CAP) return EVC_EUNSUPPORTED;
+    return EVC_OK;
+}
+
+template <int MODE>
+int proj_launch(const ProjK& k, long long lds, hipStream_t st) {
+    const dim3 grid((unsigned)(k.c.M / PG_BM), (unsigned)(k.c.Co / 64));
+    hipLaunchKernelGGL((proj_gemm_kernel<MODE>), grid, dim3(256), (size_t)lds, st, k);
+    return hipGetLastError() == hipSuccess ? EVC_OK : EVC_ELAUNCH;
+}
+
+}
+
+extern "C" int evc_proj1x1_check(const evc_proj_args* a) { return proj_validate(a); }
+
+extern "C" int evc_proj1x1_f32(const evc_proj_args* a, void* stream) {
+    const int rc = proj_validate(a);
+    if (rc != EVC_OK) return rc;
+    ProjK k{};
+    ConvK& c = k.c;
+    c.src0 = a->x; c.C0 = a->C; c.ld0 = a->ld_x ? a->ld_x : a->C;
+    c.coef_a = a->coef_a; c.coef_s = a->coef_s;
+    const char* wp = reinterpret_cast<const char*>(a->w_packed);
+    c.w = reinterpret_cast<const float*>(wp + F16_HDR_BYTES);
+    c.w_hdr = reinterpret_cast<const float*>(wp);
+    c.bias = a->bias; c.res = a->res; c.ld_res = a->ld_res; c.out_scale = a->out_scale; c.act_out = EVC_ACT_NONE;
+    c.out = a->out; c.ld_out = a->ld_out;
+    c.B = a->B; c.H = 1; c.W = a->HW; c.Co = a->Co; c.CoPad = evc_conv_co_pad(a->Co); c.KH = c.KW = 1;
+    c.M = a->B * a->HW; c.HW = a->HW; c.nchunk = a->C / KC; c.nsteps = c.nchunk; c.steps_per_split = c.nchunk; c.splits = 1;
+    c.stats = a->stats_out; c.in_bound = a->in_bound;
+    k.bound_bits = a->bound_bits; k.n_ranges = a->n_ranges; k.range_c = a->n_ranges > 0 ? a->Co / a->n_ranges : a->Co;
+    k.events = a->events; k.site_events = a->site_events ? a->site_events + a->site : nullptr;
+    const long long lds = 2LL * PG_BUF + (a->coef_a ? 8LL * a->C : 0);
+    hipStream_t st = (hipStream_t)stream;
+    return a->coef_a ? proj_launch<MODE_AFFINE>(k, lds, st) : proj_launch<MODE_PLAIN>(k, lds, st);
+}
diff --git a/extreme-video-compression-with-prediction-using-pre-trainded-diffusion-models-_amd/csrc/split_arith.h b/extreme-video-compression-with-prediction-using-pre-trainded-diffusion-models-_amd/csrc/split_arith.h
--- /dev/null
+++ b/extreme-video-compression-with-prediction-using-pre-trainded-diffusion-models-_amd/csrc/split_arith.h
@@ -0,0 +1,117 @@
+#pragma once
+#include <hip/hip_runtime.h>
+#include <stdint.h>
+#include "../../include/evc_hip.h"
+
+typedef float f32x16 __attribute__((ext_vector_type(16)));
+
+namespace {
+
+constexpr int KC = 16;
+
+constexpr int MODE_PLAIN = 0, MODE_AFFINE = 1, MODE_AFFINE_SILU = 2, MODE_SILU = 3, MODE_RELU = 4;
+
+struct ConvK {
+    const float* src0; const float* src1; int C0; int C1; int ld0; int ld1;
+    const float* coef_a; const float* coef_s;
+    const float* w; const float* bias; const float* res; int ld_res;
+    float out_scale; int act_out;
+    float* out; int ld_out;
+    int B, H, W, Co, CoPad, KH, KW;
+    int M, HW, nchunk, nsteps, steps_per_split, splits;
+    float* ws;
+    float* stats;
+    const float* w_hdr;
+    const unsigned* in_bound;
+    int tail_first, tail_splits, tail_sps, tail_rows;
+    int cut_chunk;
+    const float* x2_src0; const float* x2_src1; int x2_C0, x2_C1, x2_ld0, x2_ld1;
+    const char* x2_w;
+    const float* x2_hdr;
+    const unsigned* x2_bound;
+    int bound_stride, generic_epi;
+};
+
+__device__ __forceinline__ float bound_scale(unsigned bits) {
+    const float b = sqrtf(__uint_as_float(bits));
+    if (!(b < 3.0e38f)) return __builtin_nanf("");
+    return b > 0.f ? ldexpf(1.0f, 6 - ilogbf(b)) : 1.0f;
+}
+__device__ __forceinline__ int bound_index(const ConvK& p, int m) { return p.bound_stride ? min(m, p.M - 1) / p.HW : 0; }
+__device__ __forceinline__ float in_scale(const ConvK& p, int m) {
+    if (!p.in_bound) return 1.0f;
+    return bound_scale(p.in_bound[bound_index(p, m)]);
+}
+
+__device__ __forceinline__ float silu_f(float v) { return v * __builtin_amdgcn_rcpf(1.0f + __expf(-v)); }
+
+template <int MODE>
+__device__ __forceinline__ float4 transform(float4 v, const float4& a, const float4& s, bool ok) {
+    if (MODE == MODE_AFFINE || MODE == MODE_AFFINE_SILU) {
+        v.x = v.x * a.x + s.x; v.y = v.y * a.y + s.y; v.z = v.z * a.z + s.z; v.w = v.w * a.w + s.w;
+    }
+    if (MODE == MODE_AFFINE_SILU || MODE == MODE_SILU) {
+        v.x = silu_f(v.x); v.y = silu_f(v.y); v.z = silu_f(v.z); v.w = silu_f(v.w);
+    }
+    if (MODE == MODE_RELU) {
+        v.x = v.x < 0.f ? 0.f : v.x; v.y = v.y < 0.f ? 0.f : v.y; v.z = v.z < 0.f ? 0.f : v.z; v.w = v.w < 0.f ? 0.f : v.w;
+    }
+    v.x = ok ? v.x : 0.f; v.y = ok ? v.y : 0.f; v.z = ok ? v.z : 0.f; v.w = ok ? v.w : 0.f;
+    return v;
+}
+
+typedef __bf16 bf16x8 __attribute__((ext_vector_type(8)));
+typedef _Float16 f16x8 __attribute__((ext_vector_type(8)));
+
+__device__ __forceinline__ void split3_bf16(const float4& v0, const float4& v1, bf16x8& p1, bf16x8& p2, bf16x8& p3) {
+    const float x[8] = {v0.x, v0.y, v0.z, v0.w, v1.x, v1.y, v1.z, v1.w};
+#pragma unroll
+    for (int j = 0; j < 8; ++j) {
+        const __bf16 a = (__bf16)x[j];
+        const float r = x[j] - (float)a;
+        const __bf16 b = (__bf16)r;
+        p1[j] = a; p2[j] = b; p3[j] = (__bf16)(r - (float)b);
+    }
+}
+
+constexpr float F16_ACT_SCALE = 8.0f;
+
+__device__ __forceinline__ void split2_f16(const float4& v0, const float4& v1, float xscale, f16x8& p1, f16x8& p2) {
+    const float x[8] = {v0.x, v0.y, v0.z, v0.w, v1.x, v1.y, v1.z, v1.w};
+#pragma unroll
+    for (int j = 0; j < 8; ++j) {
+        const float v = x[j] * xscale;
+        const _Float16 a = (_Float16)v;
+        p1[j] = a; p2[j] = (_Float16)(v - (float)a);
+    }
+}
+
+template <int NP> struct Split;
+template <> struct Split<3> {
+    typedef bf16x8 vec;
+    static constexpr int NTERM = 6;
+    static __device__ __forceinline__ constexpr int qa(int t) { return t == 0 ? 2 : (t == 1 || t == 3) ? 1 : 0; }
+    static __device__ __forceinline__ constexpr int qb(int t) { return t == 2 ? 2 : (t == 1 || t == 4) ? 1 : 0; }
+    static __device__ __forceinline__ f32x16 mfma(const vec& a, const vec& b, const f32x16& c) {
+        return __builtin_amdgcn_mfma_f32_32x32x16_bf16(a, b, c, 0, 0, 0);
+    }
+    static __device__ __forceinline__ void split(const float4& v0, const float4& v1, float, vec (&pl)[3]) {
+        split3_bf16(v0, v1, pl[0], pl[1], pl[2]);
+    }
+};
+template <> struct Split<2> {
+    typedef f16x8 vec;
+    static constexpr int NTERM = 3;
+    static __device__ __forceinline__ constexpr int qa(int t) { return t == 0 ? 1 : 0; }
+    static __device__ __forceinline__ constexpr int qb(int t) { return t == 1 ? 1 : 0; }
+    static __device__ __forceinline__ f32x16 mfma(const vec& a, const vec& b, const f32x16& c) {
+        return __builtin_amdgcn_mfma_f32_32x32x16_f16(a, b, c, 0, 0, 0);
+    }
+    static __device__ __forceinline__ void split(const float4& v0, const float4& v1, float xscale, vec (&pl)[2]) {
+        split2_f16(v0, v1, xscale, pl[0], pl[1]);
+    }
+};
+
+constexpr int F16_HDR_BYTES = 256;
+
+}
diff --git a/extreme-video-compression-with-prediction-using-pre-trainded-diffusion-models-_amd/lib.py b/extreme-video-compression-with-prediction-using-pre-trainded-diffusion-models-_amd/lib.py
--- a/extreme-video-compression-with-prediction-using-pre-trainded-diffusion-models-_amd/lib.py
+++ b/extreme-video-compression-with-prediction-using-pre-trainded-diffusion-models-_amd/lib.py
@@ -59,6 +59,16 @@
     _fields_ = [("kernel", ctypes.c_char * 96), ("tile_m", c_int), ("tile_n", c_int), ("splits", c_int),
                 ("steps_per_split", c_int), ("cut_chunk", c_int), ("tail_tiles", c_int), ("tail_splits", c_int),
                 ("stats_runs", c_int), ("fused_1x1", c_int)]
+
+
+class ProjArgs(ctypes.Structure):
+    _fields_ = [("x", c_void_p), ("x1", c_void_p), ("C", c_int), ("C1", c_int), ("ld_x", c_int),
+                ("coef_a", c_void_p), ("coef_s", c_void_p), ("in_bound", c_void_p),
+                ("w_packed", c_void_p), ("arith", c_int),
+                ("bias", c_void_p), ("res", c_void_p), ("ld_res", c_int), ("out_scale", c_float),
+                ("out", c_void_p), ("ld_out", c_int), ("B", c_int), ("HW", c_int), ("Co", c_int),
+                ("stats_out", c_void_p), ("bound_bits", c_void_p), ("n_ranges", c_int),
+                ("events", c_void_p), ("site_events", c_void_p), ("site", c_int)]
 
 
 class AttentionPlan(ctypes.Structure):
@@ -144,6 +154,8 @@
     "evc_conv_workspace_bytes": (c_longlong, [POINTER(ConvArgs)]),
     "evc_conv2d_nhwc_f32": (c_int, [POINTER(ConvArgs), c_void_p, c_void_p]),
     "evc_conv2d_nhwc_profiled_f32": (c_int, [POINTER(ConvArgs), c_void_p, c_void_p, c_void_p, c_void_p]),
+    "evc_proj1x1_check": (c_int, [POINTER(ProjArgs)]),
+    "evc_proj1x1_f32": (c_int, [POINTER(ProjArgs), c_void_p]),
     "evc_attention_f32": (c_int, [c_void_p, c_void_p, c_void_p, c_int, c_void_p, c_int, c_int, c_int, c_int, c_int,
                                   c_float, c_void_p]),
     "evc_attention_workspace_bytes": (c_longlong, [c_int, c_int, c_int, c_int]),
@@ -847,6 +859,47 @@
     return result
 
 
+def proj1x1_check(B, HW, C, Co, arith, coef=False, C1=0, n_ranges=0):
+    d = c_void_p(16)
+    a = ProjArgs(x=d, x1=d if C1 else None, C=C, C1=C1, coef_a=d if coef else None, coef_s=d if coef else None, w_packed=d,
+                 arith=arith, out_scale=1.0, out=d, ld_out=Co, B=B, HW=HW, Co=Co, bound_bits=d if n_ranges else None,
+                 n_ranges=n_ranges)
+    return int(hip_lib(require_device=False).evc_proj1x1_check(ctypes.byref(a)))
+
+
+def proj1x1_supported(B, HW, C, Co, arith):
+    return proj1x1_check(B, HW, C, Co, arith) == 0
+
+
+def proj1x1(x, w_packed, Co, bias=None, coef=None, in_bound=None, res=None, out_scale=1.0, out=None, want_stats=False,
+            bound=None, site=None):
+    L = hip_lib()
+    px, C, ldx, shp = _src(x)
+    B, H, W = shp
+    dev = (x.t if isinstance(x, Cols) else x).device
+    if out is None:
+        out = torch.empty((B, H, W, Co), device=dev, dtype=torch.float32)
+    po, Cout, ldo, shpo = _src(out)
+    assert tuple(shpo) == (B, H, W) and Cout >= Co
+    pr, Cr, ldr, shpr = _src(res)
+    assert res is None or (tuple(shpr) == (B, H, W) and Cr >= Co)
+    ca, cs = coef if coef is not None else (None, None)
+    assert ca is None or (tuple(ca.shape) == (B, C) and tuple(cs.shape) == (B, C))
+    a = ProjArgs(x=px, C=C, ld_x=ldx, coef_a=ptr(ca), coef_s=ptr(cs), in_bound=_word(in_bound), w_packed=ptr(w_packed),
+                 arith=packed_arith(w_packed), bias=ptr(bias), res=pr, ld_res=ldr, out_scale=float(out_scale), out=po,
+                 ld_out=ldo, B=B, HW=H * W, Co=Co)
+    stats = None
+    if want_stats and (H * W) % 64 == 0:
+        stats = torch.empty((B, H * W // 64, Co, 2), device=dev, dtype=torch.float32)
+        a.stats_out = ptr(stats)
+    if bound is not None:
+        a.bound_bits, a.n_ranges = _word(bound, bound.numel()), bound.numel()
+        a.events, a.site_events, a.site = _site_args(site, dev)
+    _check(L.evc_proj1x1_f32(ctypes.byref(a), stream_ptr()), "evc_proj1x1_f32")
+    result = out.t if isinstance(out, Cols) else out
+    return (result, stats) if want_stats else result
+
+
 def conv_fused_stats_splits(B, H, W, Ci, Co, KH, KW, splits=0, arith=None):
     a = conv_query_args(B, H, W, Ci, 0, Co, KH, KW, default_arith() if arith is None else arith, splits=splits)
     return hip_lib(require_device=False).evc_conv_stats_splits(ctypes.byref(a))
diff --git a/extreme-video-compression-with-prediction-using-pre-trainded-diffusion-models-_amd/scorenet.py b/extreme-video-compression-with-prediction-using-pre-trainded-diffusion-models-_amd/scorenet.py
--- a/extreme-video-compression-with-prediction-using-pre-trainded-diffusion-models-_amd/scorenet.py
+++ b/extreme-video-compression-with-prediction-using-pre-trainded-diffusion-models-_amd/scorenet.py
@@ -217,6 +217,8 @@
         import os
         self.overlap_skip = os.environ.get("EVC_OVERLAP_SKIP", "1") != "0"
         self.fuse_skip = self._f16_raw and os.environ.get("EVC_FUSE_SKIP", "1") != "0"
+        self.proj_gemm = self._f16_raw and os.environ.get("EVC_PROJ_GEMM", "1") != "0"
+        self._proj_gemm_shapes = {}
         self._side_streams = {}
         self._bounds_by_stream = {}
         self._bounds = None
@@ -536,16 +538,37 @@
         coef = self._gn([x.stats()], H * W, num_groups(C), 1e-6, mode=1, gamma=e["gamma"], beta=e["beta"],
                            site=self._site("attn_norm", i))
         qkvb = self._bound_slot(3)
-        if qkvb is None:
-            obound = None
-            qkv = self._conv(x.t, e["wqkv"], 3 * C, 1, 1, bias=e["bqkv"], coef=coef)
-        else:
-            qkv, qst = self._conv(x.t, e["wqkv"], 3 * C, 1, 1, bias=e["bqkv"], coef=coef, want_stats=True)
-            self._mbound(qst, 0, C, qkvb, site=self._site("attn_qkv", i))
-            obound = _f16_only(e["wo"], qkvb.view(B, 3)[:, 2].contiguous() if self.batch_invariant else qkvb[2:3])
+        qkv, obound = self._qkv(i, e, x, coef, qkvb)
         o = self._attention(qkv.view(B, H * W, 3 * C), C, heads, bounds=None if i in self._attn_f32 else qkvb)
+        if self._proj_gemm_ok(e["wo"], B, H, W, C, C):
+            return self._act(*L.proj1x1(o.view(B, H, W, C), e["wo"], C, bias=e["bo"], in_bound=obound, res=x.t,
+                                        out_scale=INV_SQRT2, want_stats=True))
         return self._act(*self._conv(o.view(B, H, W, C), e["wo"], C, 1, 1, bias=e["bo"], res=x.t,
                                    out_scale=INV_SQRT2, want_stats=True, in_bound=obound))
+
+    def _proj_gemm_ok(self, w_packed, B, H, W, C, Co):
+        if not (self.proj_gemm and not self.batch_invariant and self._f16_raw):
+            return False
+        key = (B, H, W, C, Co, L.packed_arith(w_packed))
+        ok = self._proj_gemm_shapes.get(key)
+        if ok is None:
+            ok = L.proj1x1_supported(B, H * W, C, Co, key[5])
+            if ok:
+                plan = L.conv_plan(B, H, W, C, 0, Co, 1, key[5], coef=Co == 3 * C)
+                ok = not (plan["splits"] == 1 and plan["tile"][0] == 128)
+            self._proj_gemm_shapes[key] = ok
+        return ok
+
+    def _qkv(self, i, e, x, coef, qkvb):
+        B, H, W, C = x.t.shape
+        if qkvb is None:
+            return self._conv(x.t, e["wqkv"], 3 * C, 1, 1, bias=e["bqkv"], coef=coef), None
+        if self._proj_gemm_ok(e["wqkv"], B, H, W, C, 3 * C):
+            qkv = L.proj1x1(x.t, e["wqkv"], 3 * C, bias=e["bqkv"], coef=coef, bound=qkvb, site=self._site("attn_qkv", i))
+            return qkv, _f16_only(e["wo"], qkvb[2:3])
+        qkv, qst = self._conv(x.t, e["wqkv"], 3 * C, 1, 1, bias=e["bqkv"], coef=coef, want_stats=True)
+        self._mbound(qst, 0, C, qkvb, site=self._site("attn_qkv", i))
+        return qkv, _f16_only(e["wo"], qkvb.view(B, 3)[:, 2].contiguous() if self.batch_invariant else qkvb[2:3])
 
     @torch.no_grad()
     def forward_rows(self, x, rows, cond=None):
diff --git a/include/evc_hip.h b/include/evc_hip.h
--- a/include/evc_hip.h
+++ b/include/evc_hip.h
@@ -119,6 +119,23 @@
 
 int evc_conv2d_nhwc_profiled_f32(const evc_conv_args* a, float* ws, void* stream, void* ev_start, void* ev_conv_end);
 
+typedef struct {
+    const float* x; const float* x1; int C; int C1;
+    int ld_x;
+    const float* coef_a; const float* coef_s;
+    const unsigned* in_bound;
+    const float* w_packed; int arith;
+    const float* bias; const float* res; int ld_res;
+    float out_scale;
+    float* out; int ld_out;
+    int B; int HW; int Co;
+    float* stats_out;
+    unsigned* bound_bits; int n_ranges;
+    unsigned* events; unsigned* site_events; int site;
+} evc_proj_args;
+int evc_proj1x1_check(const evc_proj_args* a);
+int evc_proj1x1_f32(const evc_proj_args* a, void* stream);
+
 int evc_attention_f32(const float* q, const float* k, const float* v, int ld_qkv, float* out, int ld_out, int B,
                       int heads, int N, int D, float scale, void* stream);
 long long evc_attention_workspace_bytes(int B, int heads, int N, int D);
```
